# NagsTheProgrammer/WindGNN

Measured on AMD Instinct MI355X. Metric: windows/sec (fwd+bwd) 34-node seq24 GCN-GRU, higher is better.
Workload: dtype f16x3(split-fp32); 1 GPU; S=34 stations, T=24, F=13, H=102, B=4096 windows/GPU; step = forward + MSE + backward + grad all-reduce (N>1) + Adam; fp32 I/O; global_batch=4096, parallelism=dp1, math=f16x3, collective=none (one rank)

## Files before the change

### windgnn_amd/csrc/api.hip

```cpp
#include <atomic>
#include <cmath>
#include <cstdlib>
#include <mutex>

#include "common.h"
#include "../../include/windgnn_optim.h"
#include "../../include/windgnn_sched.h"

namespace {

inline size_t rup(size_t x, size_t a) { return (x + a - 1) / a * a; }

struct Layout {
  size_t BT, I, Ip, G3, Gp, H, Hp;
  size_t Id;
  int np_g3, np_i;
  size_t ws_GI, ws_g, ws_planes_f, ws_Ylast, ws_xtail_f, ws_xtail_b, fwd_floats;
  size_t st_g, st_gates, st_yp, stash_floats;
  size_t ws_dGI, ws_dGH, ws_dg, ws_part_ih, ws_part_hh, ws_gcnpart, ws_planes_b, ws_scales, ws_dY, bwd_floats;
  size_t prep_f, prep_b, prep_floats;
  int prep_kind;
  int sk_ih, sk_hh;
  bool tn_merge;
  bool x3, gen_gcn, gen_gru, g32, g32tn;
  int hq;
  int np_h;
  bool dg16;
  bool gi16;
  bool dgi1;
  bool gen2p;
  bool small, rec32;
  size_t st_hprev;
  bool dghn;
  int hn, msplit, m_hh;
  size_t st_h1;
  size_t st_stats;
  size_t st_GI;
  bool gi_stash;
  size_t ws_gh, ws_h1, ws_yp, ws_hhp_f, ws_kp_f, ws_hc, ws_du, ws_dhz, ws_dhw, ws_hhp_b, ws_kp_b, ws_dc;
  size_t ws_ntk_f, ws_ntk_b;
  size_t ws_aimg_f, ws_aimg_b;
  bool state;
  size_t plane_rows;
  size_t st_h0;
};

int pick_splitk(size_t BT, int tiles, int target_wgs, int min_rows) {
  int by_rows = (int)(BT / (size_t)min_rows);
  int by_grid = target_wgs / (tiles > 0 ? tiles : 1);
  int sk = by_rows < by_grid ? by_rows : by_grid;
  if (sk >= 8) sk -= sk % 8;
  return sk < 1 ? 1 : sk;
}

bool three_pass(const wgnn_dims* d) { return d->math == WGNN_MATH_F16X3 || d->math == WGNN_MATH_F16X3G; }

Layout make_layout(const wgnn_dims* d, bool state = false, int series = SER_NONE ) {
  Layout L;
  L.state = state;
  L.x3 = d->math != WGNN_MATH_F32;
  L.gen_gcn = d->adj_format == WGNN_ADJ_CSR;
  L.gen_gru = L.x3 ? !grux_shape_supported(d->H) : !gru_shape_supported(d->H);
  const bool x3 = L.x3;
  L.BT = (size_t)d->B * d->T;
  L.I = (size_t)d->S * d->F;
  L.Ip = rup(L.I + 1, 32);
  L.Id = rup(L.I, 16);
  L.H = d->H;
  L.Hp = x3 ? (size_t)grux_hp(d->H) : 0;
  L.G3 = 3 * (size_t)d->H;
  L.Gp = rup(L.G3, 32);
  L.np_g3 = pgemm_nt_np((int)L.G3);
  L.np_i = pgemm_nt_np((int)L.I);
  auto al = [](size_t x) { return align_up(x, 64); };
  L.g32 = !x3 && !L.gen_gcn && !L.gen_gru && gemm32_nt_supported(L.BT, (int)L.Ip, (int)L.Gp);
  L.g32tn = L.g32 && gemm32_tn_supported(L.BT);
  L.small = !x3 && !L.gen_gru && !series && gru_small_supported(d->B, d->H);
  L.rec32 = !x3 && !L.gen_gru && !L.small;
  const bool g32_shape = !x3 && !L.gen_gcn && !L.gen_gru && gemm32_nt_supported(1u << 30, (int)L.Ip, (int)L.Gp);
  const size_t planes_f = ser_front(series, x3 ? (size_t)L.np_g3 * L.Ip : (g32_shape ? (size_t)gemm32_nt_rows((int)L.G3) * L.Ip : 0));
  const size_t planes_b = ser_front(series, x3 ? (size_t)L.np_i * L.Gp : (g32_shape ? (size_t)gemm32_nt_rows((int)L.I) * L.Gp : 0));
  L.prep_kind = x3 ? 1 : (g32_shape ? 2 : 0);
  L.prep_f = 0;
  L.prep_b = al(planes_f);
  L.prep_floats = L.prep_kind ? al(planes_f) + al(planes_b) : 0;
  constexpr size_t HDR = WGNN_STATUS_BYTES / sizeof(float);
  size_t o = HDR;
  L.ws_GI = o; o += al(ser_front(series, L.BT * L.Gp));
  L.ws_g = o; o += al(ser_front(series, L.BT * L.Ip));
  L.ws_planes_f = o; o += al(planes_f);
  L.np_h = pgemm_nt_np((int)L.H);
  L.ws_gh = o; o += al(L.gen_gru ? (size_t)d->B * L.Gp : 0);
  L.ws_h1 = o; o += al(L.gen_gcn ? L.BT * L.I : 0);
  L.ws_yp = o; o += al(L.gen_gru && x3 ? (L.BT + 1) * L.Hp : 0);
  L.ws_hhp_f = o; o += al(L.gen_gru && x3 ? (size_t)L.np_g3 * L.Hp : 0);
  L.ws_kp_f = o; o += al(L.gen_gru && x3 ? pgemm_nt_kpart_floats(d->B, (int)L.Gp, (int)L.Hp) : 0);
  L.ws_hc = o; o += al(L.gen_gru && x3 ? (size_t)d->B * L.Hp : 0);
  L.ws_xtail_f = o; o += al(ser_front(series, (L.I & 1) && !L.gen_gcn ? L.I + 1 : 0));
  if ((x3 && !L.gen_gru) || L.rec32 || L.H <= L.Ip) { L.ws_Ylast = L.ws_g; }
  else { L.ws_Ylast = o; o += al(L.BT * L.H); }
  L.ws_aimg_f = o; o += al(x3 ? pgemm_nt256_aimg_bytes((int)L.BT, (int)L.G3, (int)L.Ip, 2) / 4 : 0);
  {
    const int sk = (!x3 && !L.g32 && L.BT < 65536) ? gemm_f32_nt_splitk((int)L.BT, (int)L.G3, (int)L.I) : 1;
    L.ws_ntk_f = o; o += al(ser_front(series, sk > 1 ? (size_t)sk * L.BT * L.G3 : 0));
  }
  L.fwd_floats = o;
  o = 0;
  L.st_g = o; o += al(ser_front(series, L.BT * L.Ip));
  {
    const size_t plain = L.BT * 4 * L.H, grec = (x3 && !L.gen_gru) ? grux_gates_floats(d->B, d->T, d->H, d->io)
                                                                   : (L.rec32 ? gru_gates_floats(d->B, d->T, d->H) : 0);
    L.st_gates = o; o += al(series == SER_FRONT ? 0 : series == SER_REC ? grec : (plain > grec ? plain : grec));
  }
  L.plane_rows = L.BT + (state ? (size_t)d->B : 1);
  L.st_yp = o; o += al(L.plane_rows * L.Hp);
  L.st_h1 = o; o += al(L.gen_gcn ? L.BT * L.I : 0);
  {
    const size_t nb = L.small ? (size_t)gru_small_blocks(d->B) : (size_t)grux_blocks(d->B);
    L.st_stats = o; o += al(series ? 0 : 2 * nb + 4);
  }
  L.gi_stash = (x3 && !L.gen_gru && three_pass(d)) || L.rec32;
  L.st_GI = o; o += al(ser_front(series, L.gi_stash ? L.BT * L.Gp : 0));
  L.hq = (int)rup(L.H + 1, 16);
  const bool hprev_rows = L.g32tn || (state && !x3);
  L.st_hprev = o; o += al(ser_rec(series, hprev_rows ? L.BT * (size_t)L.hq : 0));
  L.st_h0 = o; o += al(state ? (size_t)d->B * L.H : 0);
  L.stash_floats = o;
  L.dghn = (x3 && !L.gen_gru) || (L.rec32 && L.g32tn);
  L.dgi1 = d->math == WGNN_MATH_F16X3G && !L.gen_gru && L.BT >= 4096;
  L.gen2p = d->math == WGNN_MATH_F16X3G && L.gen_gru && L.BT >= 3072;
  L.dg16 = (L.dgi1 || (d->math == WGNN_MATH_F16 && !L.gen_gru)) && !L.gen_gcn;
  L.gi16 = d->math == WGNN_MATH_F16 && !L.gen_gru;
  L.hn = x3 ? grux_hn(d->H) : gru_hn(d->H);
  L.msplit = x3 ? grux_msplit(d->H) : gru_msplit(d->H);
  L.m_hh = L.dghn ? (x3 ? L.msplit + L.hn : L.msplit + (int)L.H) : (int)L.G3;
  if (x3) {
    L.sk_ih = pick_splitk(L.BT, pgemm_tn_tiles((int)L.G3, (int)L.I + 1), 256, 64);
    L.sk_hh = pick_splitk(L.BT, pgemm_tn_tiles(L.m_hh, (int)L.H + 1), 256, 64);
    L.tn_merge = L.dghn;
  } else {
    L.tn_merge = false;
    L.sk_ih = L.g32tn ? pick_splitk(L.BT, gemm32_tn_tiles((int)L.G3, (int)L.I + 1), 256, 64)
                    : pick_splitk(L.BT, gemm_f32_tiles((int)L.G3, (int)L.I + 1), 1024, 128);
    L.sk_hh = L.g32tn ? pick_splitk(L.BT, gemm32_tn_tiles(L.m_hh, (int)L.H + 1), 256, 64)
                    : pick_splitk(L.BT, gemm_f32_tiles((int)L.G3, (int)L.H + 1), 1024, 128);
  }
  size_t part_ih = (size_t)L.sk_ih * L.G3 * (L.g32tn ? (size_t)gemm32_tn_pitch((int)L.I + 1) : L.I + 1);
  size_t part_hh = (size_t)L.sk_hh * (size_t)L.m_hh * (L.g32tn ? (size_t)gemm32_tn_pitch((int)L.H + 1) : L.H + 1);
  if (x3) {
    part_ih = pgemm_tn_partial_floats((int)L.G3, (int)L.I + 1, L.sk_ih);
    part_hh = pgemm_tn_partial_floats(L.m_hh, (int)L.H + 1, L.sk_hh);
  }
  o = HDR;
  L.ws_dGI = o; o += al(L.BT * L.Gp);
  L.ws_dGH = o; o += al(ser_rec(series, L.dghn ? L.BT * (size_t)L.hn : L.BT * L.Gp));
  L.ws_dg = o; o += al(ser_front(series, L.BT * L.Id));
  L.ws_part_ih = o; o += al(ser_front(series, part_ih));
  L.ws_part_hh = o; o += al(ser_rec(series, part_hh));
  {
    size_t a = gcn32_bwd_partial_floats((int)L.BT), b = gcnx2_bwd_partial_floats((int)L.BT);
    if (L.gen_gcn) a = gcn_csr_bwd_partial_floats();
    L.ws_gcnpart = o; o += al(ser_front(series, a > b ? a : b));
  }
  L.ws_du = o; o += al(L.gen_gcn ? L.BT * L.I : 0);
  L.ws_dhz = o; o += al(L.gen_gru ? (size_t)d->B * L.H : 0);
  L.ws_dhw = o; o += al(L.gen_gru ? (size_t)d->B * L.H : 0);
  L.ws_hhp_b = o; o += al(L.gen_gru && x3 ? (size_t)L.np_h * L.Gp : 0);
  L.ws_kp_b = o; o += al(L.gen_gru && x3 ? pgemm_nt_kpart_floats(d->B, (int)L.H, (int)L.Gp) : 0);
  L.ws_dc = o; o += al(L.gen_gru && x3 ? (size_t)d->B * L.Gp : 0);
  L.ws_planes_b = o; o += al(planes_b);
  L.ws_scales = o; o += al(4096);
  L.ws_dY = o; o += al(series ? 0 : L.BT * L.H);
  L.ws_xtail_b = o; o += al(ser_front(series, (L.I & 1) && !L.gen_gcn ? L.I + 1 : 0));
  L.ws_aimg_b = o; o += al(x3 ? pgemm_nt256_aimg_bytes((int)L.BT, (int)L.I, (int)L.Gp, 2) / 4 : 0);
  {
    const int sk = (!x3 && !L.g32 && L.BT < 65536) ? gemm_f32_nt_splitk((int)L.BT, (int)L.I, (int)L.G3) : 1;
    L.ws_ntk_b = o; o += al(ser_front(series, sk > 1 ? (size_t)sk * L.BT * L.I : 0));
  }
  L.bwd_floats = o;
  return L;
}

template <class P>
void slots(const P& s, float* out[8]) {
  const float* v[8] = {s.conv1_weight, s.conv1_bias, s.conv2_weight, s.conv2_bias, s.w_ih, s.w_hh, s.b_ih, s.b_hh};
  for (int t = 0; t < 8; ++t) out[t] = const_cast<float*>(v[t]);
}

template <class P>
bool complete(const P& s, bool conv = true) {
  float* v[8];
  slots(s, v);
  for (int t = conv ? 0 : 4; t < 8; ++t)
    if (!v[t]) return false;
  return true;
}

bool overlap(const void* a, size_t na, const void* b, size_t nb) {
  return a && b && (const char*)a < (const char*)b + nb && (const char*)b < (const char*)a + na;
}

template <class Args>
void set_adam(Args& a, const wgnn_adam* adam) {
  const double bc1 = 1.0 - pow((double)adam->beta1, (double)adam->step);
  const double bc2 = 1.0 - pow((double)adam->beta2, (double)adam->step);
  a.lr_over_bc1 = (float)(adam->lr / bc1);
  a.inv_sqrt_bc2 = (float)(1.0 / sqrt(bc2));
  a.b1 = adam->beta1; a.b2 = adam->beta2; a.eps = adam->eps;
}

template <class Args>
void set_planes(Args& a, const Layout& L, void* prepared) {
  a.pf_hi = (_Float16*)((float*)prepared + L.prep_f); a.pf_lo = a.pf_hi + (size_t)L.np_g3 * L.Ip;
  a.pb_hi = (_Float16*)((float*)prepared + L.prep_b); a.pb_lo = a.pb_hi + (size_t)L.np_i * L.Gp;
  a.np_g3 = L.np_g3; a.np_i = L.np_i;
}

void fill_reduce(const Layout& L, const wgnn_dims* d, const wgnn_grads* g, float* ws, int which, FinishArgs& a) {
  a.scales = ws + L.ws_scales;
  a.status = (unsigned*)ws;
  slots(*g, a.g);
  const int F = d->F;
  const int64_t n[8] = {(int64_t)F * F, F, (int64_t)F * F, F, (int64_t)L.G3 * (int64_t)L.I, (int64_t)L.G3 * (int64_t)L.H,
                        (int64_t)L.G3, (int64_t)L.G3};
  for (int t = 0; t < 8; ++t) a.n[t] = (int)n[t];
  a.I = (int)L.I;
  if (which & 4) {
    FinSeg& ih = a.ih;
    ih.partial = ws + L.ws_part_ih;
    ih.splitk = L.sk_ih;
    ih.kind = L.x3 ? 2 : 1;
    ih.Mout = ih.Mgemm = (int)L.G3; ih.Nout = (int)L.I + 1; ih.ncols = (int)L.I;
    ih.scaled = L.x3;
    FinSeg& hh = a.hh;
    hh = ih;
    hh.partial = ws + L.ws_part_hh;
    hh.splitk = L.sk_hh;
    hh.Nout = (int)L.H + 1; hh.ncols = (int)L.H;
    hh.Mgemm = L.m_hh;
    ih.pitch = L.g32tn ? gemm32_tn_pitch(ih.Nout) : ih.Nout;
    hh.pitch = L.g32tn ? gemm32_tn_pitch(hh.Nout) : hh.Nout;
    if (L.dghn) { hh.msplit = L.msplit; hh.rows1 = 2 * d->H; }
    if (L.x3) {
      pgemm_tn_geom((int)L.G3, ih.Nout, &ih.T, &ih.nNb, &ih.ntiles);
      pgemm_tn_geom(L.m_hh, hh.Nout, &hh.T, &hh.nNb, &hh.ntiles);
    }
  }
  if (which & 2) {
    a.conv_partial = ws + L.ws_gcnpart;
    a.conv_rows = L.gen_gcn ? gcn_csr_bwd_rows()
                            : (L.x3 ? gcnx_bwd_grid((int)L.BT, d->S, three_pass(d)) : gcn32_bwd_grid((int)L.BT, d->S));
  }
}

void fill_adam(const Layout& L, const wgnn_params* p, const wgnn_adam* adam, FinishArgs& a) {
  slots(*p, a.p);
  slots(adam->exp_avg, a.m);
  slots(adam->exp_avg_sq, a.v);
  a.adam = 1;
  set_adam(a, adam);
  if (p->prepared && L.prep_kind) {
    a.prep_kind = L.prep_kind;
    if (L.prep_kind == 1) {
      set_planes(a, L, p->prepared);
    } else {
      a.wp = (float*)p->prepared + L.prep_f;
      a.wt = (float*)p->prepared + L.prep_b;
    }
    a.Ip = (int)L.Ip; a.Gp = (int)L.Gp;
  }
}

void fill_norm(const Layout& L, const wgnn_dims* d, const wgnn_grads* g, float* ws, int which, FinishArgs& a) {
  fill_reduce(L, d, g, ws, which, a);
  a.elem_mask = ((which & 4) ? 0u : 0xF0u) | ((which & 2) ? 0u : 0x0Fu);
}

size_t clip_floats(const Layout& L, const wgnn_dims* d) {
  const wgnn_grads none = {};
  float* const nowhere = reinterpret_cast<float*>((uintptr_t)WGNN_STATUS_BYTES);
  int64_t most = 0;
  for (int which = 0; which <= 6; which += 2) {
    FinishArgs a = {};
    fill_norm(L, d, &none, nowhere, which, a);
    int64_t grid;
    if (finish_grid(a, &grid) != WGNN_OK) return 0;
    most = grid > most ? grid : most;
  }
  return rup((size_t)CLIP_HDR + (size_t)most, 64);
}

std::atomic<int> g_opt[WGNN_OPT_COUNT];
std::once_flag g_opt_once;

int env_int(const char* name, int dflt, int lo, int hi) {
  const char* e = getenv(name);
  if (!e || !e[0]) return dflt;
  char* end = nullptr;
  const long v = strtol(e, &end, 10);
  return (end == e || v < lo || v > hi) ? dflt : (int)v;
}

void init_options() {
  std::call_once(g_opt_once, [] {
    for (int k = 0; k < WGNN_OPT_COUNT; ++k) g_opt[k].store(0, std::memory_order_relaxed);
    g_opt[WGNN_OPT_FUSED_FWD].store(env_int("WGNN_FUSED_FWD", 1, 0, 2), std::memory_order_relaxed);
    g_opt[WGNN_OPT_BIG_GEMM].store(1, std::memory_order_relaxed);
    g_opt[WGNN_OPT_TN_MERGED].store(1, std::memory_order_relaxed);
  });
}

int opt(int key) {
  init_options();
  return g_opt[key].load(std::memory_order_relaxed);
}

bool known_option(int key) { return key == WGNN_OPT_FUSED_FWD || key == WGNN_OPT_BIG_GEMM || key == WGNN_OPT_TN_MERGED; }

int check_dims(const wgnn_dims* d) {
  if (!d) return WGNN_ERR_NULL;
  if (d->B < 1 || d->T < 1 || d->S < 1 || d->H < 1) return WGNN_ERR_SHAPE;
  if (d->F != 13) return WGNN_ERR_SHAPE;
  if ((int64_t)d->B * d->T > (1 << 30)) return WGNN_ERR_SHAPE;
  if (d->math != WGNN_MATH_F32 && d->math != WGNN_MATH_F16X3 && d->math != WGNN_MATH_F16 && d->math != WGNN_MATH_F16X3G)
    return WGNN_ERR_DTYPE;
  if (d->io != WGNN_IO_F32 && d->io != WGNN_IO_F16 && d->io != WGNN_IO_BF16) return WGNN_ERR_DTYPE;
  if (d->io != WGNN_IO_F32 &&
      (d->math == WGNN_MATH_F32 || d->adj_format != WGNN_ADJ_DENSE || d->S > 64 || !grux_shape_supported(d->H)))
    return WGNN_ERR_UNSUPPORTED;
  if (d->adj_format == WGNN_ADJ_CSR) {
    if (d->nnz < 1 || (int64_t)d->nnz > (int64_t)d->S * d->S) return WGNN_ERR_SHAPE;
  } else if (d->adj_format == WGNN_ADJ_DENSE) {
    if (d->S > 64) return WGNN_ERR_UNSUPPORTED;
  } else {
    return WGNN_ERR_UNSUPPORTED;
  }
  if ((int64_t)3 * d->H * d->S * d->F >= (1ll << 31) || (int64_t)3 * d->H * d->H >= (1ll << 31)) return WGNN_ERR_SHAPE;
  if ((int64_t)d->B * d->T * d->S * d->F >= (1ll << 31) || (int64_t)d->B * d->T * 4 * d->H >= (1ll << 31))
    return WGNN_ERR_SHAPE;
  return WGNN_OK;
}

struct FwdCall {
  const float* A = nullptr;
  const void* X = nullptr;
  const float* g_in = nullptr;
  const wgnn_params* p = nullptr;
  const void* labels = nullptr;
  const float* h0 = nullptr;
  void* Y = nullptr;
  float* hn = nullptr;
  float* last = nullptr;
  float wind_min = 0.f, wind_max = 1.f;
  void* stash = nullptr;
  bool state = false, sst = false;
  void* workspace;
  size_t workspace_bytes;
  void* stream;
  FwdCall(void* ws, size_t ws_bytes, void* st) : workspace(ws), workspace_bytes(ws_bytes), stream(st) {}
};

struct Fwd {
  const wgnn_dims* d;
  const FwdCall& c;
  const Layout& L;
  hipStream_t st = (hipStream_t)c.stream;
  float* ws = (float*)c.workspace;
  unsigned* status = (unsigned*)c.workspace;
  float* sf = (float*)c.stash;
  float* GI = (sf && L.gi_stash) ? sf + L.st_GI : ws + L.ws_GI;
  float* g = sf ? sf + L.st_g : ws + L.ws_g;
  float* gates = sf ? sf + L.st_gates : nullptr;
  bool full = three_pass(d);
  bool kept = c.p->prepared != nullptr && L.prep_kind != 0;
  float* img_f = kept ? (float*)c.p->prepared + L.prep_f : ws + L.ws_planes_f;
  bool reg = (L.x3 && !L.gen_gru) || L.rec32;
  void* Y = (!reg && (c.last || (c.state && !c.Y))) ? ws + L.ws_Ylast : c.Y;
};

int fwd_front(const Fwd& f) {
  const wgnn_dims* d = f.d;
  const FwdCall& c = f.c;
  const Layout& L = f.L;
  const wgnn_params* p = c.p;
  const int fmode = opt(WGNN_OPT_FUSED_FWD);
  int rc;
  if (c.g_in) {
    rc = launch_pack_g(c.g_in, L.BT, (int)L.I, f.g, (int)L.Ip, f.st);
  } else if (L.x3 && !L.gen_gcn && !L.gen_gru && (fmode == 2 || (fmode == 1 && !f.sf)) && gcngi_supported(d->S, d->H, f.full)) {
    const int planes = f.sf ? ((f.full && !L.dgi1) ? 2 : 1) : 0;
    return launch_gcngi_fwd((int)L.BT, d->S, c.A, c.X, d->io, p->conv1_weight, p->conv1_bias, p->conv2_weight, p->conv2_bias,
                            f.sf ? (void*)f.g : nullptr, (int)L.Ip, planes, f.img_f, L.np_g3, f.GI, (int)L.Gp, (int)L.G3, f.full,
                            f.status, f.ws + L.ws_xtail_f, f.st);
  } else if (L.gen_gcn) {
    rc = launch_gcn2_csr_fwd((int)L.BT, d->S, d->nnz, c.A, (const float*)c.X, p->conv1_weight, p->conv1_bias, p->conv2_weight,
                             p->conv2_bias, f.sf ? f.sf + L.st_h1 : f.ws + L.ws_h1, L.x3 ? nullptr : f.g, L.x3 ? f.g : nullptr,
                             L.Ip, f.full, L.x3 ? f.status : nullptr, f.st);
  } else if (L.x3) {
    rc = launch_gcnx2_fwd((int)L.BT, d->S, c.A, c.X, d->io, p->conv1_weight, p->conv1_bias, p->conv2_weight, p->conv2_bias, f.g,
                          (int)L.Ip, f.full, f.status, f.ws + L.ws_xtail_f, f.st);
  } else {
    rc = launch_gcn32_fwd((int)L.BT, d->S, c.A, (const float*)c.X, p->conv1_weight, p->conv1_bias, p->conv2_weight,
                          p->conv2_bias, f.g, (int)L.Ip, f.ws + L.ws_xtail_f, f.st);
  }
  if (rc != WGNN_OK) return rc;
  if (L.x3) {
    const _Float16* ghi = (const _Float16*)f.g;
    const size_t aimg_f = pgemm_nt256_aimg_bytes((int)L.BT, (int)L.G3, (int)L.Ip, 2);
    return launch_pgemm_nt(ghi, ghi + L.BT * L.Ip, (int)L.Ip, (int)L.BT, (int)L.Ip, f.img_f, L.np_g3, f.GI, (int)L.Gp,
                           (int)L.G3, nullptr, f.full, nullptr, f.st, L.gi16, aimg_f ? f.ws + L.ws_aimg_f : nullptr);
  }
  if (L.g32) {
    if (!f.kept) {
      rc = launch_pad_weight(p->w_ih, (int)L.G3, (int)L.I, 0, p->b_ih, f.img_f, gemm32_nt_rows((int)L.G3), (int)L.Ip, f.st);
      if (rc != WGNN_OK) return rc;
    }
    return launch_gemm32_nt(f.g, (int)L.Ip, (int)L.BT, (int)L.Ip, f.img_f, f.GI, (int)L.Gp, (int)L.G3, f.st);
  }
  GemmArgs ga = {};
  ga.A = f.g; ga.lda = (int)L.Ip; ga.a_kcontig = 1;
  ga.B = p->w_ih; ga.ldb = (int)L.I; ga.b_kcontig = 1;
  ga.C = f.GI; ga.ldc = (int)L.Gp; ga.M = (int)L.BT; ga.N = (int)L.G3; ga.K = (int)L.I;
  ga.bias = p->b_ih; ga.splitk = 1;
  return launch_gemm_f32_nt(ga, gemm_f32_nt_splitk(ga.M, ga.N, ga.K) > 1 && L.BT < 65536 ? f.ws + L.ws_ntk_f : nullptr, f.st);
}

int fwd_recurrence(const Fwd& f) {
  const wgnn_dims* d = f.d;
  const FwdCall& c = f.c;
  const Layout& L = f.L;
  const wgnn_params* p = c.p;
  const float y_mul = c.wind_max - c.wind_min, y_add = c.wind_min;
  const bool hn_only = c.state && !f.Y;
  float* Y = (float*)f.Y;
  const void* labels = f.sf ? c.labels : nullptr;
  float* stats = f.sf ? f.sf + L.st_stats : nullptr;
  float* hprev = (f.sf && (L.g32tn || c.sst)) ? f.sf + L.st_hprev : nullptr;
  int rc;
  if (L.x3 && !L.gen_gru) {
    if (c.last)
      return launch_grux_fwd(d->B, d->T, d->H, f.GI, (int)L.Gp, p->w_hh, p->b_hh, c.last, nullptr, nullptr, f.full, f.status,
                             nullptr, nullptr, 0, 1, y_mul, y_add, f.st);
    if (c.state) {
      const int lo = hn_only && d->io == WGNN_IO_F32;
      return launch_grux_fwd(d->B, d->T, d->H, f.GI, (int)L.Gp, p->w_hh, p->b_hh, lo ? (void*)c.hn : f.Y, nullptr, nullptr,
                             f.full, f.status, nullptr, nullptr, d->io, lo, 1.f, 0.f, f.st, c.h0, lo ? nullptr : c.hn);
    }
    rc = launch_grux_fwd(d->B, d->T, d->H, f.GI, (int)L.Gp, p->w_hh, p->b_hh, f.Y, f.gates,
                         f.sf && !hh_from_y(d, L.tn_merge, c.sst) ? f.sf + L.st_yp : nullptr, f.full, f.status, labels, stats,
                         d->io, 0, 1.f, 0.f, f.st, c.h0, c.hn, c.sst ? L.plane_rows : 0);
  } else if (L.rec32) {
    if (c.last)
      return launch_gru_fwd(d->B, d->T, d->H, f.GI, (int)L.Gp, p->w_hh, p->b_hh, c.last, nullptr, nullptr, nullptr, nullptr, 0,
                            1, y_mul, y_add, f.st);
    if (c.state)
      return launch_gru_fwd(d->B, d->T, d->H, f.GI, (int)L.Gp, p->w_hh, p->b_hh, hn_only ? c.hn : Y, nullptr, nullptr, nullptr,
                            nullptr, 0, hn_only ? 1 : 0, 1.f, 0.f, f.st, c.h0, hn_only ? nullptr : c.hn);
    rc = launch_gru_fwd(d->B, d->T, d->H, f.GI, (int)L.Gp, p->w_hh, p->b_hh, Y, f.gates, (const float*)labels, stats, hprev,
                        L.hq, 0, 1.f, 0.f, f.st, c.h0, c.hn);
  } else if (L.small) {
    rc = launch_gru_small_fwd(d->B, d->T, d->H, f.GI, (int)L.Gp, p->w_hh, p->b_hh, Y, f.gates, hprev, L.hq,
                              (const float*)labels, stats, f.st, c.h0, c.hn);
  } else if (L.x3) {
    rc = launch_split_weight2(p->w_hh, (int)L.G3, (int)L.H, 0, p->b_hh, (int)L.H, f.ws + L.ws_hhp_f, L.np_g3, (int)L.Hp,
                              f.status, f.st);
    if (rc == WGNN_OK)
      rc = launch_gru_gen_fwd_x3(d->B, d->T, d->H, f.GI, (int)L.Gp, f.ws + L.ws_hhp_f, L.np_g3, p->b_hh, Y, f.gates,
                                 f.sf ? f.sf + L.st_yp : f.ws + L.ws_yp, f.ws + L.ws_gh, f.ws + L.ws_kp_f, f.ws + L.ws_hc,
                                 f.full, f.st, c.h0, c.sst ? L.plane_rows : 0);
  } else {
    rc = launch_gru_gen_fwd(d->B, d->T, d->H, f.GI, (int)L.Gp, p->w_hh, p->b_hh, Y, f.gates, f.ws + L.ws_gh, f.st, c.h0);
  }
  if (rc != WGNN_OK) return rc;
  const size_t h4 = (size_t)d->H * 4;
  if (L.gen_gru && c.hn &&
      hipMemcpy2DAsync(c.hn, h4, Y + (size_t)(d->T - 1) * d->H, d->T * h4, h4, d->B, hipMemcpyDeviceToDevice, f.st) != hipSuccess)
    return WGNN_ERR_HIP;
  if (c.sst) {
    const float* h0c = f.sf + L.st_h0;
    if (L.x3) {
      _Float16* yh = (_Float16*)(f.sf + L.st_yp);
      return launch_h0_planes(d->B, d->H, (int)L.Hp, h0c, yh + L.BT * L.Hp, yh + (L.plane_rows + L.BT) * L.Hp, f.st);
    }
    float* hp = f.sf + L.st_hprev;
    const size_t hq4 = (size_t)L.hq * 4;
    if (L.gen_gru && L.BT > 1 &&
        hipMemcpy2DAsync(hp + L.hq, hq4, Y, h4, h4, L.BT - 1, hipMemcpyDeviceToDevice, f.st) != hipSuccess)
      return WGNN_ERR_HIP;
    return hipMemcpy2DAsync(hp, (size_t)d->T * hq4, h0c, h4, h4, d->B, hipMemcpyDeviceToDevice, f.st) == hipSuccess ? WGNN_OK
                                                                                                              : WGNN_ERR_HIP;
  }
  if (c.last)
    return wgnn_predict_last(Y, d->B, d->T, d->H, c.wind_min, c.wind_max, c.last, c.stream);
  return WGNN_OK;
}

int fwd(const wgnn_dims* d, const FwdCall& c) {
  int rc = check_dims(d);
  if (rc != WGNN_OK) return rc;
  if ((!c.g_in && (!c.A || !c.X)) || !c.p || (!c.Y && !c.last && !(c.state && c.hn)) || (c.sst && !c.stash) || !c.workspace)
    return WGNN_ERR_NULL;
  if (!complete(*c.p, !c.g_in)) return WGNN_ERR_NULL;
  if (c.g_in && (d->math != WGNN_MATH_F32 || d->io != WGNN_IO_F32 || d->adj_format != WGNN_ADJ_DENSE)) return WGNN_ERR_UNSUPPORTED;
  const size_t hb = (size_t)d->B * d->H * sizeof(float), yb = (size_t)d->B * d->T * d->H * (d->io == WGNN_IO_F32 ? 4 : 2);
  if (overlap(c.h0, hb, c.hn, hb) || overlap(c.h0, hb, c.Y, yb) || overlap(c.Y, yb, c.hn, hb)) return WGNN_ERR_UNSUPPORTED;
  const Layout L = make_layout(d, c.sst);
  if (c.workspace_bytes < sizeof(float) * L.fwd_floats) return WGNN_ERR_WORKSPACE;
  const wgnn_params* p = c.p;
  hipStream_t st = (hipStream_t)c.stream;
  if (c.state && d->T == 1 && d->adj_format == WGNN_ADJ_DENSE && d->io == WGNN_IO_F32 && gru_step_supported(d->B, d->S, d->H))
    return launch_gru_step(d->B, d->S, d->H, c.A, (const float*)c.X, p->conv1_weight, p->conv1_bias, p->conv2_weight,
                           p->conv2_bias, p->w_ih, p->b_ih, p->w_hh, p->b_hh, c.h0, (float*)c.Y, c.hn, st);
  const Fwd f{d, c, L};
  if (c.sst &&
      (c.h0 ? hipMemcpyAsync(f.sf + L.st_h0, c.h0, hb, hipMemcpyDeviceToDevice, st)
            : hipMemsetAsync(f.sf + L.st_h0, 0, hb, st)) != hipSuccess)
    return WGNN_ERR_HIP;
  if (L.x3 && !f.kept) {
    rc = launch_split_weight2(p->w_ih, (int)L.G3, (int)L.I, 0, p->b_ih, (int)L.I, f.img_f, L.np_g3, (int)L.Ip, f.status, st);
    if (rc != WGNN_OK) return rc;
  }
  rc = fwd_front(f);
  if (rc != WGNN_OK) return rc;
  return fwd_recurrence(f);
}

struct BwdCall {
  const float* A = nullptr;
  const void* X = nullptr;
  const wgnn_params* p = nullptr;
  const void* Y = nullptr;
  const float* dY = nullptr;
  const void* labels = nullptr;
  float grad_scale = 1.f;
  float* loss = nullptr;
  const void* stash = nullptr;
  const wgnn_grads* g = nullptr;
  int part = 0;
  float* dg_out = nullptr;
  bool sst = false;
  const float* dhn = nullptr;
  float* dh0 = nullptr;
  void* workspace;
  size_t workspace_bytes;
  void* stream;
  BwdCall(void* ws, size_t ws_bytes, void* st) : workspace(ws), workspace_bytes(ws_bytes), stream(st) {}
};

struct Bwd {
  const wgnn_dims* d;
  const BwdCall& c;
  const Layout& L;
  hipStream_t st = (hipStream_t)c.stream;
  float* ws = (float*)c.workspace;
  unsigned* status = (unsigned*)c.workspace;
  const float* sf = (const float*)c.stash;
  const float* Y = (const float*)c.Y;
  const float* gact = sf + L.st_g;
  float* dGI = ws + L.ws_dGI;
  float* dGH = ws + L.ws_dGH;
  float* dg = ws + L.ws_dg;
  float* scales = ws + L.ws_scales;
  bool full = three_pass(d);
  bool defer = c.part & WGNN_BWD_DEFER;
  bool stats_ready = (c.part & 8) && c.labels;
  bool fused_loss = c.labels && ((L.x3 && !L.gen_gru) || ((L.rec32 || L.small) && stats_ready));
};

int bwd_rec(const Bwd& b) {
  const wgnn_dims* d = b.d;
  const BwdCall& c = b.c;
  const Layout& L = b.L;
  const wgnn_params* p = c.p;
  const float* labels = (const float*)c.labels;
  const float* gates = b.sf + L.st_gates;
  const float* stats = b.fused_loss && b.stats_ready ? b.sf + L.st_stats : nullptr;
  const BwdState sbs = {c.sst ? b.sf + L.st_h0 : nullptr, c.dhn, c.dh0};
  const BwdState* sb = c.sst ? &sbs : nullptr;
  const float* dY = c.dY;
  int rc;
  if (labels && !b.fused_loss) {
    rc = launch_mse(b.Y, labels, (int64_t)L.BT * L.H, c.grad_scale, b.ws + L.ws_dY, c.loss, b.scales + 64, b.st);
    if (rc != WGNN_OK) return rc;
    dY = b.ws + L.ws_dY;
  }
  if (L.x3) {
    if (b.fused_loss && b.stats_ready)
      rc = WGNN_OK;
    else if (b.fused_loss)
      rc = launch_mse_stats(b.Y, labels, (int64_t)L.BT * L.H, c.grad_scale, c.loss, b.scales, b.scales + 64, b.st);
    else
      rc = launch_amax_scale(dY, (int64_t)L.BT * L.H, b.scales, b.scales + 64, b.st,
                             c.dhn, c.dhn ? (int64_t)d->B * d->H : 0);
    if (rc != WGNN_OK) return rc;
    if (L.gen_gru) {
      rc = launch_split_weight2(p->w_hh, (int)L.G3, (int)L.H, 1, nullptr, 0, b.ws + L.ws_hhp_b, L.np_h, (int)L.Gp, b.status,
                                b.st);
      if (rc != WGNN_OK) return rc;
      return launch_gru_gen_bwd_x3(d->B, d->T, d->H, b.ws + L.ws_hhp_b, L.np_h, b.Y, dY, gates, b.scales, b.dGI, b.dGH,
                                   (int)L.Gp, b.ws + L.ws_dhz, b.ws + L.ws_dhw, b.ws + L.ws_kp_b, b.ws + L.ws_dc, b.full, b.st, sb);
    }
    return launch_grux_bwd(d->B, d->T, d->H, p->w_hh, c.Y, b.fused_loss ? nullptr : dY, b.fused_loss ? c.labels : nullptr,
                           d->io, gates, L.gi_stash ? b.sf + L.st_GI : nullptr, (int)L.Gp, b.scales, b.dGI, b.dGH, (int)L.Gp,
                           b.full, stats, (int64_t)L.BT * L.H, c.grad_scale, c.loss, b.scales, b.status, L.dgi1 ? 0 : 1, b.st,
                           sb);
  }
  if (L.gen_gru)
    return launch_gru_gen_bwd(d->B, d->T, d->H, p->w_hh, b.Y, dY, gates, b.dGI, b.dGH, (int)L.Gp, b.ws + L.ws_dhz,
                              b.ws + L.ws_dhw, b.st, sb);
  if (L.small)
    return launch_gru_small_bwd(d->B, d->T, d->H, p->w_hh, b.Y, b.fused_loss ? nullptr : dY, b.fused_loss ? labels : nullptr,
                                gates, b.dGI, b.dGH, (int)L.Gp, stats, (int64_t)L.BT * L.H, c.grad_scale, c.loss, b.status,
                                b.st, sb);
  return launch_gru_bwd(d->B, d->T, d->H, p->w_hh, b.Y, b.fused_loss ? nullptr : dY, b.fused_loss ? labels : nullptr, gates,
                        b.sf + L.st_GI, (int)L.Gp, b.dGI, (int)L.Gp, L.dghn ? b.dGH : nullptr, L.dghn ? nullptr : b.dGH, stats,
                        (int64_t)L.BT * L.H, c.grad_scale, c.loss, b.status, b.st, sb);
}

int bwd_weights(const Bwd& b, int prods, int r0, int rows) {
  const wgnn_dims* d = b.d;
  const Layout& L = b.L;
  float* part_ih = b.ws + L.ws_part_ih;
  float* part_hh = b.ws + L.ws_part_hh;
  const bool sst = b.c.sst;
  int rc = WGNN_OK;
  if (L.x3) {
    const _Float16* dGIh = (const _Float16*)b.dGI + r0;
    const _Float16* dGHh = (const _Float16*)b.dGH + r0;
    const _Float16* gh = (const _Float16*)b.gact;
    const _Float16 *yph = (const _Float16*)(b.sf + L.st_yp), *ypl = yph + L.plane_rows * L.Hp;
    const size_t PG = L.BT * L.Gp;
    TnProd hh = {};
    hh.lda = (int)L.Gp; hh.Bhi = yph; hh.Blo = ypl; hh.ldb = (int)L.Hp; hh.shift_T = d->T; hh.splitk = L.sk_hh;
    hh.partial = part_hh; hh.Nout = (int)L.H + 1; hh.x3 = b.full; hh.per_window = sst;
    if (L.dghn) {
      hh.Ahi = dGIh; hh.Alo = L.dgi1 ? nullptr : dGIh + PG; hh.Mout = L.m_hh;
      hh.A2hi = dGHh; hh.A2lo = L.dgi1 ? nullptr : dGHh + L.BT * (size_t)L.hn; hh.lda2 = L.hn; hh.msplit = L.msplit;
      hh.b_stream = true;
    } else {
      hh.Ahi = dGHh; hh.Alo = L.gen2p ? nullptr : dGHh + PG; hh.Mout = rows;
    }
    const bool one_pass_ih = L.dgi1 || L.gen2p;
    TnProd ih = {};
    ih.Ahi = dGIh; ih.Alo = one_pass_ih ? dGIh : dGIh + PG; ih.lda = (int)L.Gp;
    ih.Bhi = gh; ih.Blo = gh + L.BT * L.Ip; ih.ldb = (int)L.Ip; ih.splitk = L.sk_ih;
    ih.partial = part_ih; ih.Mout = rows; ih.Nout = (int)L.I + 1; ih.x3 = b.full && !one_pass_ih; ih.b_stream = true;
    auto one = [&](const TnProd& p) {
      return launch_pgemm_tn(p.Ahi, p.Alo, p.lda, p.Bhi, p.Blo, p.ldb, p.shift_T, (int)L.BT, p.splitk, p.partial, p.Mout, p.Nout,
                             p.x3, p.A2hi, p.A2lo, p.lda2, p.msplit, b.st, p.b_stream, p.per_window);
    };
    if (prods == (WGNN_ROWS_IH | WGNN_ROWS_HH) && L.tn_merge && opt(WGNN_OPT_TN_MERGED) && pgemm_tn2_covers(ih, hh)) {
      rc = launch_pgemm_tn2(ih, tn_b_from_y(hh, hh_from_y(d, L.tn_merge, sst) ? b.Y : nullptr, (int)L.H), (int)L.BT, b.st);
    } else {
      if (prods & WGNN_ROWS_HH) {
        rc = one(hh);
        if (rc != WGNN_OK) return rc;
      }
      if (prods & WGNN_ROWS_IH) rc = one(ih);
    }
  } else {
    const float* hp = b.sf + L.st_hprev;
    if (prods & WGNN_ROWS_HH) {
      if (L.g32tn && L.dghn)
        rc = launch_gemm32_tn(b.dGI, (int)L.Gp, hp, L.hq, (int)L.BT, L.sk_hh, part_hh, L.m_hh, (int)L.H + 1, b.dGH, L.hn,
                              L.msplit, b.st);
      else if (L.g32tn)
        rc = launch_gemm32_tn(b.dGH, (int)L.Gp, hp, L.hq, (int)L.BT, L.sk_hh, part_hh, rows, (int)L.H + 1, nullptr, 0, 0, b.st);
      else {
        GemmArgs a = {};
        a.A = b.dGH + r0; a.lda = (int)L.Gp; a.a_kcontig = 0;
        a.B = b.Y; a.ldb = (int)L.H; a.b_kcontig = 0; a.ones_col = 1; a.shift_T = d->T;
        if (sst) { a.B = hp; a.ldb = L.hq; a.shift_T = 0; }
        a.M = rows; a.N = (int)L.H + 1; a.K = (int)L.BT;
        a.splitk = L.sk_hh; a.partial = part_hh;
        rc = launch_gemm_f32(a, b.st);
      }
      if (rc != WGNN_OK) return rc;
    }
    if (prods & WGNN_ROWS_IH) {
      if (L.g32tn) {
        rc = launch_gemm32_tn(b.dGI, (int)L.Gp, b.gact, (int)L.Ip, (int)L.BT, L.sk_ih, part_ih, rows, (int)L.I + 1, nullptr, 0,
                              0, b.st);
      } else {
        GemmArgs a = {};
        a.A = b.dGI + r0; a.lda = (int)L.Gp; a.a_kcontig = 0;
        a.B = b.gact; a.ldb = (int)L.Ip; a.b_kcontig = 0; a.ones_col = 1;
        a.M = rows; a.N = (int)L.I + 1; a.K = (int)L.BT;
        a.splitk = L.sk_ih; a.partial = part_ih;
        rc = launch_gemm_f32(a, b.st);
      }
    }
  }
  if (rc != WGNN_OK || b.defer) return rc;
  FinishArgs a = {};
  fill_reduce(L, d, b.c.g, b.ws, 4, a);
  if (prods != (WGNN_ROWS_IH | WGNN_ROWS_HH)) {
    const bool ih = prods == WGNN_ROWS_IH;
    FinSeg& s = ih ? a.ih : a.hh;
    (ih ? a.hh : a.ih) = FinSeg{};
    if (rows != (int)L.G3) {
      s.Mout = s.Mgemm = rows;
      if (L.x3) pgemm_tn_geom(rows, s.Nout, &s.T, &s.nNb, &s.ntiles);
    }
    a.g[ih ? 4 : 5] += (size_t)r0 * s.ncols;
    a.g[ih ? 6 : 7] += r0;
  }
  return launch_finish(a, b.st);
}

int bwd_dg(const Bwd& b) {
  const wgnn_dims* d = b.d;
  const BwdCall& c = b.c;
  const Layout& L = b.L;
  const wgnn_params* p = c.p;
  const bool kept = p->prepared != nullptr && L.prep_kind != 0;
  float* img_b = kept ? (float*)p->prepared + L.prep_b : b.ws + L.ws_planes_b;
  int rc;
  if (L.x3) {
    if (!kept) {
      rc = launch_split_weight2(p->w_ih, (int)L.G3, (int)L.I, 1, nullptr, 0, img_b, L.np_i, (int)L.Gp, b.status, b.st);
      if (rc != WGNN_OK) return rc;
    }
    const _Float16* dGIh = (const _Float16*)b.dGI;
    const size_t aimg_b = pgemm_nt256_aimg_bytes((int)L.BT, (int)L.I, (int)L.Gp, 2);
    rc = launch_pgemm_nt(dGIh, (L.dgi1 || L.gen2p) ? nullptr : dGIh + L.BT * L.Gp, (int)L.Gp, (int)L.BT, (int)L.Gp, img_b,
                         L.np_i, b.dg, (int)L.Id, (int)L.I, nullptr, b.full, nullptr, b.st, L.dg16,
                         aimg_b ? b.ws + L.ws_aimg_b : nullptr);
  } else if (L.g32) {
    if (!kept) {
      rc = launch_pad_weight(p->w_ih, (int)L.G3, (int)L.I, 1, nullptr, img_b, gemm32_nt_rows((int)L.I), (int)L.Gp, b.st);
      if (rc != WGNN_OK) return rc;
    }
    rc = launch_gemm32_nt(b.dGI, (int)L.Gp, (int)L.BT, (int)L.Gp, img_b, b.dg, (int)L.Id, (int)L.I, b.st);
  } else {
    GemmArgs a = {};
    a.A = b.dGI; a.lda = (int)L.Gp; a.a_kcontig = 1;
    a.B = p->w_ih; a.ldb = (int)L.I; a.b_kcontig = 0;
    a.C = b.dg; a.ldc = (int)L.Id; a.M = (int)L.BT; a.N = (int)L.I; a.K = (int)L.G3; a.splitk = 1;
    rc = launch_gemm_f32_nt(a, gemm_f32_nt_splitk(a.M, a.N, a.K) > 1 && L.BT < 65536 ? b.ws + L.ws_ntk_b : nullptr, b.st);
  }
  if (rc != WGNN_OK) return rc;
  if (c.dg_out) return launch_unpack_dg(b.dg, L.BT, (int)L.I, (int)L.Id, c.dg_out, b.st);
  if (L.gen_gcn)
    rc = launch_gcn2_csr_bwd((int)L.BT, d->S, d->nnz, c.A, (const float*)c.X, p->conv2_weight, b.sf + L.st_h1,
                             L.x3 ? nullptr : b.gact, L.x3 ? b.gact : nullptr, L.Ip, b.dg, L.Id, L.x3 ? b.scales : nullptr,
                             b.ws + L.ws_du, b.ws + L.ws_gcnpart, nullptr, nullptr, nullptr, nullptr, b.st);
  else if (L.x3)
    rc = launch_gcnx2_bwd((int)L.BT, d->S, c.A, c.X, d->io, p->conv1_weight, p->conv1_bias, p->conv2_weight, b.gact, (int)L.Ip,
                          b.dg, (int)L.Id, L.dg16, b.scales, 0, b.ws + L.ws_gcnpart, b.full, b.ws + L.ws_xtail_b,
                          b.st);
  else
    rc = launch_gcn32_bwd((int)L.BT, d->S, c.A, (const float*)c.X, p->conv1_weight, p->conv1_bias, p->conv2_weight, b.gact,
                          (int)L.Ip, b.dg, (int)L.Id, nullptr, nullptr, nullptr, nullptr, b.ws + L.ws_gcnpart,
                          b.ws + L.ws_xtail_b, b.st);
  if (rc != WGNN_OK || b.defer) return rc;
  FinishArgs a = {};
  fill_reduce(L, d, c.g, b.ws, 2, a);
  return launch_finish(a, b.st);
}

int bwd(const wgnn_dims* d, const BwdCall& c) {
  const int which = c.part;
  if (which < 1 || which > 31 || (which & 7) == 0) return WGNN_ERR_SHAPE;
  int rc = check_dims(d);
  if (rc != WGNN_OK) return rc;
  if ((!c.dg_out && (!c.A || !c.X)) || !c.p || !c.Y || (!c.dY && !c.labels) || !c.stash || !c.g || !c.workspace)
    return WGNN_ERR_NULL;
  if (c.labels && (which & 1) && !c.loss) return WGNN_ERR_NULL;
  if (!complete(*c.g, !c.dg_out)) return WGNN_ERR_NULL;
  if (c.dg_out && (d->math != WGNN_MATH_F32 || d->io != WGNN_IO_F32 || d->adj_format != WGNN_ADJ_DENSE || which != 7))
    return WGNN_ERR_UNSUPPORTED;
  const Layout L = make_layout(d, c.sst);
  if (c.workspace_bytes < sizeof(float) * L.bwd_floats) return WGNN_ERR_WORKSPACE;
  const Bwd b{d, c, L};
  if (d->io != WGNN_IO_F32 && c.labels && (which & 1) && !(b.fused_loss && b.stats_ready)) return WGNN_ERR_UNSUPPORTED;
  if (which & 1) {
    rc = bwd_rec(b);
    if (rc != WGNN_OK) return rc;
  }
  if (which & 4) {
    rc = bwd_weights(b, WGNN_ROWS_IH | WGNN_ROWS_HH, 0, (int)L.G3);
    if (rc != WGNN_OK) return rc;
  }
  return (which & 2) ? bwd_dg(b) : WGNN_OK;
}

int rows_align(const wgnn_dims* d, const Layout& L) {
  if (!L.gen_gru || d->math == WGNN_MATH_F16) return 0;
  return L.x3 ? TN_BM : 128;
}

int check_rows(const wgnn_dims* d, const Layout& L, int which, int row0, int rows) {
  if ((which & ~(WGNN_ROWS_IH | WGNN_ROWS_HH | WGNN_ROWS_STATE)) != 0 ||
      ((which & 3) != WGNN_ROWS_IH && (which & 3) != WGNN_ROWS_HH))
    return WGNN_ERR_SHAPE;
  if (which & WGNN_ROWS_STATE) return WGNN_ERR_UNSUPPORTED;
  const int al = rows_align(d, L);
  if (al == 0) return WGNN_ERR_UNSUPPORTED;
  const int64_t end = (int64_t)row0 + rows;
  if (row0 < 0 || rows < 1 || end > (int64_t)L.G3 || row0 % al != 0 || (end % al != 0 && end != (int64_t)L.G3))
    return WGNN_ERR_SHAPE;
  return WGNN_OK;
}

}

int opt_big_gemm() { return opt(WGNN_OPT_BIG_GEMM); }

bool hh_from_y(const wgnn_dims* d, bool tn_merge, bool sst) {
  static const int from_env = env_int("WGNN_TN_YFP32", 1, 0, 1);
  return tn_merge && three_pass(d) && d->io == WGNN_IO_F32 && !sst && from_env && opt(WGNN_OPT_TN_MERGED);
}

int series_plan(const wgnn_dims* df, const wgnn_dims* dr, SeriesPlan* sp) {
  int rc = check_dims(df);
  if (rc == WGNN_OK) rc = check_dims(dr);
  if (rc != WGNN_OK) return rc;
  const Layout Lf = make_layout(df, false, SER_FRONT), Lr = make_layout(dr, false, SER_REC);
  if ((int64_t)Lf.BT * (int64_t)Lf.Gp >= (1ll << 31)) return WGNN_ERR_SHAPE;
  sp->ws_front = Lf.fwd_floats > Lf.bwd_floats ? Lf.fwd_floats : Lf.bwd_floats;
  sp->ws_rec = Lr.fwd_floats > Lr.bwd_floats ? Lr.fwd_floats : Lr.bwd_floats;
  sp->ws_front_fwd = Lf.fwd_floats;
  sp->st_front = Lf.stash_floats;
  sp->st_rec = Lr.stash_floats;
  sp->st_g = Lf.BT * Lf.Ip; sp->st_GI = Lf.BT * Lf.Gp;
  sp->st_gates = gru_gates_floats(dr->B, dr->T, dr->H);
  sp->st_hprev = Lr.g32tn ? Lr.BT * (size_t)Lr.hq : 0;
  return WGNN_OK;
}

namespace {

int series_forward(const wgnn_dims* df, const wgnn_dims* dr, int stride, const float* A, const float* Xs, const wgnn_params* p,
                   float* Y, float* last, float wind_min, float wind_max, void* stash, void* workspace, const SeriesPlan& sp,
                   void* stream, const float* Ls, int64_t ls_rows, float* loss_buf, const int* starts, bool masked = false,
                   const LossFn* lossfn = nullptr) {
  const int last_start = df->T - dr->T;
  const Layout Lf = make_layout(df, false, SER_FRONT), Lr = make_layout(dr, false, SER_REC);
  FwdCall cf(workspace, sizeof(float) * sp.ws_front, stream);
  cf.A = A; cf.X = Xs; cf.p = p; cf.stash = stash;
  const Fwd f{df, cf, Lf};
  int rc = fwd_front(f);
  if (rc != WGNN_OK) return rc;
  hipStream_t st = (hipStream_t)stream;
  const int ld = (int)Lf.Gp;
  if (last)
    return launch_gru_fwd(dr->B, dr->T, dr->H, f.GI, ld, p->w_hh, p->b_hh, last, nullptr, nullptr, nullptr, nullptr, 0, 1,
                          wind_max - wind_min, wind_min, st, nullptr, nullptr, stride, 0, starts, last_start);
  float* sr = stash ? (float*)stash + sp.st_front : nullptr;
  return launch_gru_fwd(dr->B, dr->T, dr->H, f.GI, ld, p->w_hh, p->b_hh, Y, sr ? sr + Lr.st_gates : nullptr, Ls, loss_buf,
                        sr && Lr.g32tn ? sr + Lr.st_hprev : nullptr, Lr.hq, 0, 1.f, 0.f, st, nullptr, nullptr, stride, ls_rows,
                        starts, last_start, masked, lossfn);
}

int series_backward(const wgnn_dims* df, const wgnn_dims* dr, int stride, const float* A, const float* Xs, const wgnn_params* p,
                    const float* Y, const float* dY, const void* stash, const wgnn_grads* g, void* workspace, const SeriesPlan& sp,
                    void* stream, const float* Ls, int64_t ls_rows, float grad_scale, const float* loss_buf, float* loss,
                    const int* starts, bool masked = false, const LossFn* lossfn = nullptr) {
  const Layout Lf = make_layout(df, false, SER_FRONT), Lr = make_layout(dr, false, SER_REC);
  const float* sff = (const float*)stash;
  BwdCall cr((float*)workspace + sp.ws_front, sizeof(float) * sp.ws_rec, stream);
  cr.p = p; cr.Y = Y; cr.dY = dY; cr.stash = sff + sp.st_front; cr.g = g; cr.part = 7;
  const Bwd br{dr, cr, Lr};
  BwdCall cf(workspace, sizeof(float) * sp.ws_front, stream);
  cf.A = A; cf.X = Xs; cf.p = p; cf.Y = Y; cf.dY = dY; cf.stash = stash; cf.g = g; cf.part = 7;
  const Bwd bf{df, cf, Lf};
  int rc = launch_gru_bwd(dr->B, dr->T, dr->H, p->w_hh, Y, dY, Ls, br.sf + Lr.st_gates, sff + Lf.st_GI, (int)Lf.Gp, br.dGI,
                          (int)Lr.Gp, Lr.dghn ? br.dGH : nullptr, Lr.dghn ? nullptr : br.dGH, loss_buf, (int64_t)Lr.BT * Lr.H,
                          grad_scale, loss, Ls ? br.status : nullptr, br.st, nullptr, stride, ls_rows, starts,
                          df->T - dr->T, masked, lossfn);
  if (rc != WGNN_OK) return rc;
  rc = bwd_weights(br, WGNN_ROWS_HH, 0, (int)Lr.G3);
  if (rc != WGNN_OK) return rc;
  rc = starts ? launch_series_fold_at(br.dGI, starts, dr->B, dr->T, df->T, (int)Lf.G3, (int)Lf.Gp, bf.dGI, bf.st)
              : launch_series_fold(br.dGI, dr->B, dr->T, stride, df->T, (int)Lf.G3, (int)Lf.Gp, bf.dGI, bf.st);
  if (rc != WGNN_OK) return rc;
  rc = bwd_weights(bf, WGNN_ROWS_IH, 0, (int)Lf.G3);
  if (rc != WGNN_OK) return rc;
  return bwd_dg(bf);
}

}

int series_fwd(const wgnn_dims* df, const wgnn_dims* dr, int stride, const float* A, const float* Xs, const wgnn_params* p,
               float* Y, float* last, float wind_min, float wind_max, void* stash, void* workspace, const SeriesPlan& sp,
               void* stream, const int* starts) {
  return series_forward(df, dr, stride, A, Xs, p, Y, last, wind_min, wind_max, stash, workspace, sp, stream, nullptr, 0, nullptr,
                        starts);
}

int series_bwd(const wgnn_dims* df, const wgnn_dims* dr, int stride, const float* A, const float* Xs, const wgnn_params* p,
               const float* Y, const float* dY, const void* stash, const wgnn_grads* g, void* workspace, const SeriesPlan& sp,
               void* stream, const int* starts) {
  return series_backward(df, dr, stride, A, Xs, p, Y, dY, stash, g, workspace, sp, stream, nullptr, 0, 1.f, nullptr, nullptr,
                         starts);
}

size_t series_loss_floats(int n) { return 2 * (size_t)gru_blocks(n) + 4; }
size_t series_masked_loss_floats(int n) { return series_loss_floats(n) + (size_t)gru_blocks(n); }

int series_fwd_loss(const wgnn_dims* df, const wgnn_dims* dr, int stride, const float* A, const float* Xs, const wgnn_params* p,
                    const float* Ls, int64_t ls_rows, float* Y, void* stash, float* loss_buf, void* workspace,
                    const SeriesPlan& sp, void* stream, const int* starts, bool masked, const LossFn* lossfn) {
  return series_forward(df, dr, stride, A, Xs, p, Y, nullptr, 0.f, 1.f, stash, workspace, sp, stream, Ls, ls_rows, loss_buf,
                        starts, masked, lossfn);
}

int series_bwd_mse(const wgnn_dims* df, const wgnn_dims* dr, int stride, const float* A, const float* Xs, const wgnn_params* p,
                   const float* Y, const float* Ls, int64_t ls_rows, float grad_scale, const void* stash, const float* loss_buf,
                   float* loss, const wgnn_grads* g, void* workspace, const SeriesPlan& sp, void* stream, const int* starts,
                   bool masked, const LossFn* lossfn) {
  return series_backward(df, dr, stride, A, Xs, p, Y, nullptr, stash, g, workspace, sp, stream, Ls, ls_rows, grad_scale, loss_buf,
                         loss, starts, masked, lossfn);
}

int series_val_fwd(const wgnn_dims* df, const wgnn_dims* dr, int stride, const float* A, const float* Xs, const wgnn_params* p,
                   const float* Ls, int64_t ls_rows, float* last, float wind_min, float wind_max, float* loss_buf,
                   void* workspace, const SeriesPlan& sp, void* stream, const int* starts, const LossFn* lossfn) {
  const Layout Lf = make_layout(df, false, SER_FRONT);
  FwdCall cf(workspace, sizeof(float) * sp.ws_front_fwd, stream);
  cf.A = A; cf.X = Xs; cf.p = p;
  const Fwd f{df, cf, Lf};
  int rc = fwd_front(f);
  if (rc != WGNN_OK) return rc;
  return launch_gru_fwd(dr->B, dr->T, dr->H, f.GI, (int)Lf.Gp, p->w_hh, p->b_hh, last, nullptr, Ls, loss_buf, nullptr, 0, 1,
                        wind_max - wind_min, wind_min, (hipStream_t)stream, nullptr, nullptr, stride, ls_rows, starts,
                        df->T - dr->T, false, lossfn);
}

extern "C" {

int wgnn_version(void) { return WGNN_VERSION; }

int wgnn_get_option(int key) { return known_option(key) ? opt(key) : WGNN_ERR_SHAPE; }

int wgnn_set_option(int key, int value) {
  if (!known_option(key)) return WGNN_ERR_SHAPE;
  if (key == WGNN_OPT_FUSED_FWD && (value < 0 || value > 2)) return WGNN_ERR_SHAPE;
  if ((key == WGNN_OPT_BIG_GEMM || key == WGNN_OPT_TN_MERGED) && (value < 0 || value > 1)) return WGNN_ERR_SHAPE;
  init_options();
  return g_opt[key].exchange(value, std::memory_order_relaxed);
}

const char* wgnn_strerror(int status) {
  switch (status) {
    case WGNN_OK: return "ok";
    case WGNN_ERR_NULL: return "required pointer is NULL";
    case WGNN_ERR_SHAPE: return "invalid shape (need B,T,S,H >= 1 and F == 13)";
    case WGNN_ERR_DTYPE: return "unsupported dtype / math mode";
    case WGNN_ERR_WORKSPACE: return "workspace or stash too small";
    case WGNN_ERR_UNSUPPORTED:
      return "configuration not supported by this build (a dense adjacency needs S <= 64: pass larger graphs as CSR)";
    case WGNN_ERR_HIP: return "HIP runtime error (kernel launch failed)";
    case WGNN_ERR_RANGE:
      return "a value left fp16's range in an fp16-plane math mode (status block bits: 1 activation, 2 weight, 4 "
             "non-finite gradient): normalise the inputs or use WGNN_MATH_F32; or (bit 8) the backward was told the "
             "forward's loss statistics are in the stash but the last forward on it was not wgnn_fwd_loss";
    default: return "unknown status";
  }
}

size_t wgnn_workspace_bytes(const wgnn_dims* d) {
  if (check_dims(d) != WGNN_OK) return 0;
  Layout L = make_layout(d);
  return sizeof(float) * (L.fwd_floats > L.bwd_floats ? L.fwd_floats : L.bwd_floats);
}

size_t wgnn_stash_bytes(const wgnn_dims* d) {
  if (check_dims(d) != WGNN_OK) return 0;
  return sizeof(float) * make_layout(d).stash_floats;
}

size_t wgnn_state_stash_bytes(const wgnn_dims* d) {
  if (check_dims(d) != WGNN_OK) return 0;
  return sizeof(float) * make_layout(d, true).stash_floats;
}

size_t wgnn_prepared_bytes(const wgnn_dims* d) {
  if (check_dims(d) != WGNN_OK) return 0;
  return sizeof(float) * make_layout(d).prep_floats;
}

int wgnn_fwd(const wgnn_dims* d, const float* A, const void* X, const wgnn_params* p, void* Y, void* stash,
             void* workspace, size_t workspace_bytes, void* stream) {
  FwdCall c(workspace, workspace_bytes, stream);
  c.A = A; c.X = X; c.p = p; c.Y = Y; c.stash = stash;
  return fwd(d, c);
}

int wgnn_fwd_loss(const wgnn_dims* d, const float* A, const void* X, const wgnn_params* p, const void* labels,
                  void* Y, void* stash, void* workspace, size_t workspace_bytes, void* stream) {
  if (!labels || !stash) return WGNN_ERR_NULL;
  FwdCall c(workspace, workspace_bytes, stream);
  c.A = A; c.X = X; c.p = p; c.labels = labels; c.Y = Y; c.stash = stash;
  return fwd(d, c);
}

int wgnn_fwd_last(const wgnn_dims* d, const float* A, const void* X, const wgnn_params* p, float wind_min,
                  float wind_max, float* out, void* workspace, size_t workspace_bytes, void* stream) {
  if (!out) return WGNN_ERR_NULL;
  if (d && d->io != WGNN_IO_F32) return WGNN_ERR_UNSUPPORTED;
  FwdCall c(workspace, workspace_bytes, stream);
  c.A = A; c.X = X; c.p = p; c.last = out; c.wind_min = wind_min; c.wind_max = wind_max;
  return fwd(d, c);
}

int wgnn_fwd_state(const wgnn_dims* d, const float* A, const void* X, const wgnn_params* p, const float* h0, void* Y,
                   float* h_n, void* workspace, size_t workspace_bytes, void* stream) {
  FwdCall c(workspace, workspace_bytes, stream);
  c.A = A; c.X = X; c.p = p; c.h0 = h0; c.Y = Y; c.hn = h_n; c.state = true;
  return fwd(d, c);
}

int wgnn_fwd_state_stash(const wgnn_dims* d, const float* A, const void* X, const wgnn_params* p, const float* h0, void* Y,
                         float* h_n, void* stash, void* workspace, size_t workspace_bytes, void* stream) {
  FwdCall c(workspace, workspace_bytes, stream);
  c.A = A; c.X = X; c.p = p; c.h0 = h0; c.Y = Y; c.hn = h_n; c.stash = stash; c.sst = true;
  return fwd(d, c);
}

int wgnn_gru_fwd(const wgnn_dims* d, const float* g, const wgnn_params* p, void* Y, void* stash, void* workspace,
                 size_t workspace_bytes, void* stream) {
  if (!g) return WGNN_ERR_NULL;
  FwdCall c(workspace, workspace_bytes, stream);
  c.g_in = g; c.p = p; c.Y = Y; c.stash = stash;
  return fwd(d, c);
}

int wgnn_prepare_weights(const wgnn_dims* d, const wgnn_params* p, void* workspace, size_t workspace_bytes,
                         void* stream) {
  int rc = check_dims(d);
  if (rc != WGNN_OK) return rc;
  if (!p || !p->w_ih || !p->b_ih || !p->prepared || !workspace) return WGNN_ERR_NULL;
  if (workspace_bytes < WGNN_STATUS_BYTES) return WGNN_ERR_WORKSPACE;
  const Layout L = make_layout(d);
  if (L.prep_kind == 0) return WGNN_ERR_UNSUPPORTED;
  hipStream_t st = (hipStream_t)stream;
  float* img_f = (float*)p->prepared + L.prep_f;
  float* img_b = (float*)p->prepared + L.prep_b;
  if (L.prep_kind == 1) {
    rc = launch_split_weight2(p->w_ih, (int)L.G3, (int)L.I, 0, p->b_ih, (int)L.I, img_f, L.np_g3, (int)L.Ip,
                              (unsigned*)workspace, st);
    if (rc != WGNN_OK) return rc;
    return launch_split_weight2(p->w_ih, (int)L.G3, (int)L.I, 1, nullptr, 0, img_b, L.np_i, (int)L.Gp, (unsigned*)workspace, st);
  }
  rc = launch_pad_weight(p->w_ih, (int)L.G3, (int)L.I, 0, p->b_ih, img_f, gemm32_nt_rows((int)L.G3), (int)L.Ip, st);
  if (rc != WGNN_OK) return rc;
  return launch_pad_weight(p->w_ih, (int)L.G3, (int)L.I, 1, nullptr, img_b, gemm32_nt_rows((int)L.I), (int)L.Gp, st);
}

int wgnn_bwd(const wgnn_dims* d, const float* A, const void* X, const wgnn_params* p, const void* Y,
             const float* dY, const void* stash, const wgnn_grads* g, void* workspace, size_t workspace_bytes,
             void* stream) {
  return wgnn_bwd_part(d, A, X, p, Y, dY, stash, g, workspace, workspace_bytes, stream, 7);
}

int wgnn_bwd_part(const wgnn_dims* d, const float* A, const void* X, const wgnn_params* p, const void* Y,
                  const float* dY, const void* stash, const wgnn_grads* g, void* workspace, size_t workspace_bytes,
                  void* stream, int which) {
  if (!dY) return WGNN_ERR_NULL;
  BwdCall c(workspace, workspace_bytes, stream);
  c.A = A; c.X = X; c.p = p; c.Y = Y; c.dY = dY; c.stash = stash; c.g = g; c.part = which;
  return bwd(d, c);
}

int wgnn_bwd_mse_part(const wgnn_dims* d, const float* A, const void* X, const wgnn_params* p, const void* Y,
                      const void* labels, float grad_scale, float* loss, const void* stash, const wgnn_grads* g,
                      void* workspace, size_t workspace_bytes, void* stream, int which) {
  if (!labels) return WGNN_ERR_NULL;
  BwdCall c(workspace, workspace_bytes, stream);
  c.A = A; c.X = X; c.p = p; c.Y = Y; c.labels = labels; c.grad_scale = grad_scale; c.loss = loss; c.stash = stash; c.g = g;
  c.part = which;
  return bwd(d, c);
}

int wgnn_bwd_state_part(const wgnn_dims* d, const float* A, const void* X, const wgnn_params* p, const void* Y,
                        const float* dY, const float* dh_n, const void* stash, const wgnn_grads* g, float* dh0,
                        void* workspace, size_t workspace_bytes, void* stream, int part) {
  int rc = check_dims(d);
  if (rc != WGNN_OK) return rc;
  if (!dY) return WGNN_ERR_NULL;
  const size_t hb = (size_t)d->B * d->H * sizeof(float), yb = (size_t)d->B * d->T * d->H * sizeof(float);
  if (overlap(dh0, hb, dh_n, hb) || overlap(dh0, hb, dY, yb) || overlap(dh0, hb, stash, wgnn_state_stash_bytes(d)))
    return WGNN_ERR_UNSUPPORTED;
  BwdCall c(workspace, workspace_bytes, stream);
  c.A = A; c.X = X; c.p = p; c.Y = Y; c.dY = dY; c.stash = stash; c.g = g; c.part = part;
  c.sst = true; c.dhn = dh_n; c.dh0 = dh0;
  return bwd(d, c);
}

int wgnn_gru_bwd(const wgnn_dims* d, const float* g, const wgnn_params* p, const void* Y, const float* dY, const void* stash,
                 const wgnn_grads* grads, float* dg, void* workspace, size_t workspace_bytes, void* stream) {
  if (!g || !dY || !dg) return WGNN_ERR_NULL;
  BwdCall c(workspace, workspace_bytes, stream);
  c.p = p; c.Y = Y; c.dY = dY; c.stash = stash; c.g = grads; c.part = 7; c.dg_out = dg;
  return bwd(d, c);
}

int wgnn_bwd_rows_align(const wgnn_dims* d) {
  if (check_dims(d) != WGNN_OK) return 0;
  return rows_align(d, make_layout(d));
}

int wgnn_bwd_rows(const wgnn_dims* d, const void* Yv, const void* stash, const wgnn_grads* g, int which, int row0, int rows,
                  void* workspace, size_t workspace_bytes, void* stream) {
  int rc = check_dims(d);
  if (rc != WGNN_OK) return rc;
  if (!Yv || !stash || !g || !workspace) return WGNN_ERR_NULL;
  const bool ih = (which & 3) == WGNN_ROWS_IH;
  if (ih ? (!g->w_ih || !g->b_ih) : (!g->w_hh || !g->b_hh)) return WGNN_ERR_NULL;
  const Layout L = make_layout(d);
  rc = check_rows(d, L, which, row0, rows);
  if (rc != WGNN_OK) return rc;
  if (workspace_bytes < sizeof(float) * L.bwd_floats) return WGNN_ERR_WORKSPACE;
  BwdCall c(workspace, workspace_bytes, stream);
  c.Y = Yv; c.stash = stash; c.g = g;
  return bwd_weights(Bwd{d, c, L}, which & 3, row0, rows);
}

int wgnn_finish(const wgnn_dims* d, const wgnn_params* p, const wgnn_grads* g, int which, const wgnn_adam* adam,
                void* workspace, size_t workspace_bytes, void* stream) {
  int rc = check_dims(d);
  if (rc != WGNN_OK) return rc;
  const int only = which & (WGNN_FINISH_ADAM_GRU | WGNN_FINISH_ADAM_CONV);
  if ((which & ~(6 | WGNN_FINISH_ADAM_GRU | WGNN_FINISH_ADAM_CONV)) != 0 || (which == 0 && !adam)) return WGNN_ERR_SHAPE;
  if (only && (!adam || (which & 6) != 0 || only == (WGNN_FINISH_ADAM_GRU | WGNN_FINISH_ADAM_CONV))) return WGNN_ERR_SHAPE;
  if (!g || !workspace || (adam && !p)) return WGNN_ERR_NULL;
  if (!complete(*g)) return WGNN_ERR_NULL;
  const Layout L = make_layout(d);
  if (workspace_bytes < sizeof(float) * L.bwd_floats) return WGNN_ERR_WORKSPACE;
  FinishArgs a = {};
  fill_reduce(L, d, g, (float*)workspace, which, a);
  if (adam) {
    if (!complete(*p)) return WGNN_ERR_NULL;
    if (adam->step < 1) return WGNN_ERR_SHAPE;
    if (!complete(adam->exp_avg) || !complete(adam->exp_avg_sq)) return WGNN_ERR_NULL;
    fill_adam(L, p, adam, a);
    a.elem_mask = ((which & 4) ? 0u : 0xF0u) | ((which & 2) ? 0u : 0x0Fu);
    if (only == WGNN_FINISH_ADAM_GRU) a.elem_mask = 0xF0u;
    if (only == WGNN_FINISH_ADAM_CONV) a.elem_mask = 0x0Fu;
  }
  return launch_finish(a, (hipStream_t)stream);
}

int wgnn_optim_version(void) { return WGNN_OPTIM_VERSION; }

int wgnn_tn_split(const wgnn_dims* d, int state, wgnn_tn_split_info* out) {
  int rc = check_dims(d);
  if (rc != WGNN_OK) return rc;
  if (!out) return WGNN_ERR_NULL;
  const Layout L = make_layout(d, state != 0);
  out->sk_ih = L.sk_ih;
  out->sk_hh = L.sk_hh;
  out->kchunk_ih = cdiv_i(cdiv_i((int)L.BT, L.sk_ih), 32) * 32;
  out->kchunk_hh = cdiv_i(cdiv_i((int)L.BT, L.sk_hh), 32) * 32;
  out->merged = L.tn_merge ? 1 : 0;
  out->workgroups = 0;
  if (L.x3) {
    const int ni = L.sk_ih * pgemm_tn_tiles((int)L.G3, (int)L.I + 1), nh = L.sk_hh * pgemm_tn_tiles(L.m_hh, (int)L.H + 1);
    out->workgroups = L.tn_merge ? (ni > nh ? ni : nh) : ni + nh;
  }
  return WGNN_OK;
}

size_t wgnn_clip_bytes(const wgnn_dims* d) {
  if (check_dims(d) != WGNN_OK) return 0;
  return sizeof(float) * clip_floats(make_layout(d), d);
}

int wgnn_finish_norm(const wgnn_dims* d, const wgnn_grads* g, int which, float max_norm, void* clip, void* workspace,
                     size_t workspace_bytes, void* stream) {
  int rc = check_dims(d);
  if (rc != WGNN_OK) return rc;
  if ((which & ~6) != 0 || !(max_norm > 0.f)) return WGNN_ERR_SHAPE;
  if (!g || !clip || !workspace) return WGNN_ERR_NULL;
  if (!complete(*g)) return WGNN_ERR_NULL;
  const Layout L = make_layout(d);
  if (workspace_bytes < sizeof(float) * L.bwd_floats) return WGNN_ERR_WORKSPACE;
  FinishArgs a = {};
  fill_norm(L, d, g, (float*)workspace, which, a);
  a.clip = (float*)clip;
  a.max_norm = max_norm;
  int64_t grid;
  if (finish_grid(a, &grid) != WGNN_OK || (size_t)CLIP_HDR + (size_t)grid > clip_floats(L, d)) return WGNN_ERR_SHAPE;
  return launch_finish_norm(a, (hipStream_t)stream);
}

int wgnn_finish_clipped(const wgnn_dims* d, const wgnn_params* p, const wgnn_grads* g, const wgnn_adam* adam, const void* clip,
                        void* workspace, size_t workspace_bytes, void* stream) {
  int rc = check_dims(d);
  if (rc != WGNN_OK) return rc;
  if (!p || !g || !adam || !clip || !workspace) return WGNN_ERR_NULL;
  if (!complete(*g) || !complete(*p) || !complete(adam->exp_avg) || !complete(adam->exp_avg_sq)) return WGNN_ERR_NULL;
  if (adam->step < 1) return WGNN_ERR_SHAPE;
  const Layout L = make_layout(d);
  if (workspace_bytes < sizeof(float) * L.bwd_floats) return WGNN_ERR_WORKSPACE;
  FinishArgs a = {};
  fill_norm(L, d, g, (float*)workspace, 0, a);
  fill_adam(L, p, adam, a);
  a.clip = const_cast<float*>((const float*)clip);
  return launch_finish_clipped(a, (hipStream_t)stream);
}

int wgnn_finish_rows(const wgnn_dims* d, const wgnn_params* p, const wgnn_grads* g, int which, int row0, int rows,
                     const wgnn_adam* adam, void* workspace, size_t workspace_bytes, void* stream) {
  int rc = check_dims(d);
  if (rc != WGNN_OK) return rc;
  if (!p || !g || !adam || !workspace) return WGNN_ERR_NULL;
  const Layout L = make_layout(d);
  rc = check_rows(d, L, which, row0, rows);
  if (rc != WGNN_OK) return rc;
  if (adam->step < 1) return WGNN_ERR_SHAPE;
  if (workspace_bytes < WGNN_STATUS_BYTES) return WGNN_ERR_WORKSPACE;
  const bool ih = (which & 3) == WGNN_ROWS_IH;
  const wgnn_grads& m = adam->exp_avg;
  const wgnn_grads& v = adam->exp_avg_sq;
  RowsAdamArgs r = {};
  r.ncols = ih ? (int)L.I : (int)L.H;
  const size_t off = (size_t)row0 * r.ncols;
  r.p_w = const_cast<float*>(ih ? p->w_ih : p->w_hh);
  r.m_w = ih ? m.w_ih : m.w_hh;
  r.v_w = ih ? v.w_ih : v.w_hh;
  r.g_w = ih ? g->w_ih : g->w_hh;
  r.p_b = const_cast<float*>(ih ? p->b_ih : p->b_hh);
  r.m_b = ih ? m.b_ih : m.b_hh;
  r.v_b = ih ? v.b_ih : v.b_hh;
  r.g_b = ih ? g->b_ih : g->b_hh;
  if (!r.p_w || !r.m_w || !r.v_w || !r.g_w || !r.p_b || !r.m_b || !r.v_b || !r.g_b) return WGNN_ERR_NULL;
  r.p_w += off; r.m_w += off; r.v_w += off; r.g_w += off;
  r.p_b += row0; r.m_b += row0; r.v_b += row0; r.g_b += row0;
  r.row0 = row0;
  r.rows = rows;
  set_adam(r, adam);
  r.status = (unsigned*)workspace;
  if (ih && p->prepared && L.prep_kind == 1) set_planes(r, L, p->prepared);
  return launch_adam_rows(r, (hipStream_t)stream);
}

static int gcn_layer_route(int32_t ntiles, int32_t S, int32_t F, int32_t F_out, bool* wide) {
  if (ntiles < 1 || S < 1 || F < 1 || F_out < 1) return WGNN_ERR_SHAPE;
  *wide = F > 64 || F_out > 64;
  if (*wide && !gcn_wide_countable(ntiles, S, F, F_out)) return WGNN_ERR_SHAPE;
  if (!(*wide ? gcn_wide_supported(S, F, F_out) : gcn_any_supported(S, F, F_out))) return WGNN_ERR_UNSUPPORTED;
  return WGNN_OK;
}

size_t wgnn_gcn_layer_workspace_bytes(int32_t ntiles, int32_t S, int32_t F, int32_t F_out) {
  bool wide = false;
  if (gcn_layer_route(ntiles, S, F, F_out, &wide) != WGNN_OK) return 0;
  if (wide) return sizeof(float) * gcn_wide_bwd_ws_floats(ntiles, S, F, F_out);
  if (F == 13 && F_out == 13) return sizeof(float) * gcn1_bwd_partial_floats(ntiles);
  return sizeof(float) * gcn_any_bwd_partial_floats(ntiles, F, F_out);
}

int wgnn_gcn_layer_fwd(int32_t ntiles, int32_t S, int32_t F, int32_t F_out, const float* A, const float* X, const float* W,
                       const float* b, float* out, void* stream) {
  bool wide = false;
  const int rc = gcn_layer_route(ntiles, S, F, F_out, &wide);
  if (rc != WGNN_OK) return rc;
  if (!A || !X || !W || !b || !out) return WGNN_ERR_NULL;
  if (wide) return launch_gcn_wide_fwd(ntiles, S, F, F_out, A, X, W, b, out, (hipStream_t)stream);
  if (F == 13 && F_out == 13) return launch_gcn1_fwd(ntiles, S, A, X, W, b, out, (hipStream_t)stream);
  return launch_gcn_any_fwd(ntiles, S, F, F_out, A, X, W, b, out, (hipStream_t)stream);
}

int wgnn_gcn_layer_bwd(int32_t ntiles, int32_t S, int32_t F, int32_t F_out, const float* A, const float* X, const float* W,
                       const float* out, const float* dout, float* dW, float* db, float* dX, void* workspace,
                       size_t workspace_bytes, void* stream) {
  bool wide = false;
  const int rc = gcn_layer_route(ntiles, S, F, F_out, &wide);
  if (rc != WGNN_OK) return rc;
  if (!A || !X || !W || !out || !dout || !dW || !db || !workspace) return WGNN_ERR_NULL;
  if (workspace_bytes < wgnn_gcn_layer_workspace_bytes(ntiles, S, F, F_out)) return WGNN_ERR_WORKSPACE;
  if (wide)
    return launch_gcn_wide_bwd(ntiles, S, F, F_out, A, X, W, out, dout, dW, db, dX, (float*)workspace, (hipStream_t)stream);
  if (F == 13 && F_out == 13)
    return launch_gcn1_bwd(ntiles, S, A, X, W, out, dout, dW, db, dX, (float*)workspace, (hipStream_t)stream);
  return launch_gcn_any_bwd(ntiles, S, F, F_out, A, X, W, out, dout, dW, db, dX, (float*)workspace, (hipStream_t)stream);
}

size_t wgnn_gcn_layer_csr_workspace_bytes(int32_t ntiles, int32_t S, int32_t F) {
  if (ntiles < 1 || S < 1 || F != 13 || (int64_t)ntiles * S * F >= (1ll << 31)) return 0;
  return sizeof(float) * gcn1_csr_bwd_ws_floats(ntiles, S);
}

int wgnn_gcn_layer_csr_fwd(int32_t ntiles, int32_t S, int32_t F, int32_t nnz, const void* csr, const float* X,
                           const float* W, const float* b, float* out, void* stream) {
  if (ntiles < 1 || S < 1 || F != 13 || nnz < 1 || (int64_t)ntiles * S * F >= (1ll << 31)) return WGNN_ERR_SHAPE;
  if (!csr || !X || !W || !b || !out) return WGNN_ERR_NULL;
  return launch_gcn1_csr_fwd(ntiles, S, nnz, csr, X, W, b, out, (hipStream_t)stream);
}

int wgnn_gcn_layer_csr_bwd(int32_t ntiles, int32_t S, int32_t F, int32_t nnz, const void* csr, const float* X,
                           const float* W, const float* out, const float* dout, float* dW, float* db, float* dX,
                           void* workspace, size_t workspace_bytes, void* stream) {
  if (ntiles < 1 || S < 1 || F != 13 || nnz < 1 || (int64_t)ntiles * S * F >= (1ll << 31)) return WGNN_ERR_SHAPE;
  if (!csr || !X || !W || !out || !dout || !dW || !db || !workspace) return WGNN_ERR_NULL;
  if (workspace_bytes < wgnn_gcn_layer_csr_workspace_bytes(ntiles, S, F)) return WGNN_ERR_WORKSPACE;
  return launch_gcn1_csr_bwd(ntiles, S, nnz, csr, X, W, out, dout, dW, db, dX, (float*)workspace, (hipStream_t)stream);
}

int wgnn_mse_loss_grad(const float* Y, const float* L, int64_t n, float grad_scale, float* dY, float* loss,
                       void* workspace, size_t workspace_bytes, void* stream) {
  if (!Y || !L || !loss || !workspace) return WGNN_ERR_NULL;
  if (n < 1) return WGNN_ERR_SHAPE;
  if (workspace_bytes < 4096) return WGNN_ERR_WORKSPACE;
  return launch_mse(Y, L, n, grad_scale, dY, loss, (float*)workspace, (hipStream_t)stream);
}

int wgnn_adam_step(float* param, const float* grad, float* exp_avg, float* exp_avg_sq, int64_t n, int32_t step,
                   float lr, float beta1, float beta2, float eps, void* stream) {
  if (!param || !grad || !exp_avg || !exp_avg_sq) return WGNN_ERR_NULL;
  if (n < 1 || step < 1) return WGNN_ERR_SHAPE;
  return launch_adam(param, grad, exp_avg, exp_avg_sq, n, step, lr, beta1, beta2, eps, (hipStream_t)stream);
}

}
```

### windgnn_amd/csrc/common.h

```cpp
#pragma once
#include <hip/hip_runtime.h>
#include <stdint.h>

#include "../../include/windgnn.h"

typedef float f32x4 __attribute__((ext_vector_type(4)));
typedef float f32x16 __attribute__((ext_vector_type(16)));

#define WGNN_WAVE 64

static inline int cdiv_i(int a, int b) { return (a + b - 1) / b; }
static inline size_t align_up(size_t x, size_t a) { return (x + a - 1) / a * a; }

#define WGNN_CHECK_LAUNCH()                              \
  do {                                                   \
    if (hipGetLastError() != hipSuccess) return WGNN_ERR_HIP; \
  } while (0)

__device__ __forceinline__ f32x4 mfma16(float a, float b, f32x4 c) {
  return __builtin_amdgcn_mfma_f32_16x16x4f32(a, b, c, 0, 0, 0);
}
__device__ __forceinline__ f32x16 mfma32(float a, float b, f32x16 c) {
  return __builtin_amdgcn_mfma_f32_32x32x2f32(a, b, c, 0, 0, 0);
}

__device__ __forceinline__ float sigmoidf_(float x) { return 1.0f / (1.0f + expf(-x)); }
__device__ __forceinline__ float sigmoid_fast(float x) {
  return __builtin_amdgcn_rcpf(1.0f + __builtin_amdgcn_exp2f(-1.4426950408889634f * x));
}
__device__ __forceinline__ float tanh_fast(float x) {
  return 1.0f - 2.0f * __builtin_amdgcn_rcpf(__builtin_amdgcn_exp2f(2.8853900817779268f * x) + 1.0f);
}
__device__ __forceinline__ float tanhf_(float x) {
  return 1.0f - 2.0f / (expf(2.0f * x) + 1.0f);
}

#include <atomic>
static inline int ensure_dyn_smem(const void* fn, size_t bytes, std::atomic<unsigned long long>& done) {
  int dev = 0;
  if (hipGetDevice(&dev) != hipSuccess) return WGNN_ERR_HIP;
  const unsigned long long bit = 1ull << (dev & 63);
  if (done.load(std::memory_order_acquire) & bit) return WGNN_OK;
  if (hipFuncSetAttribute(fn, hipFuncAttributeMaxDynamicSharedMemorySize, (int)bytes) != hipSuccess)
    return WGNN_ERR_HIP;
  done.fetch_or(bit, std::memory_order_release);
  return WGNN_OK;
}

void prof_begin(const char* kernel, double flops, double bytes, hipStream_t st);
void prof_end(hipStream_t st);
extern bool g_prof_on;
#define PROF_LAUNCH(name, flops, bytes, st, ...) \
  do {                                            \
    if (g_prof_on) prof_begin(name, flops, bytes, st); \
    __VA_ARGS__;                                  \
    if (g_prof_on) prof_end(st);                  \
  } while (0)

#define WGNN_FP16_MAX 65504.0f
__device__ __forceinline__ bool out_of_fp16_range(float v) { return !(__builtin_fabsf(v) <= WGNN_FP16_MAX); }
__device__ __forceinline__ void report_status(unsigned* status, bool bad, unsigned bit) {
  if (status && bad) atomicOr(status, bit);
}

struct BwdState { const float* h0; const float* dhn; float* dh0; };
template <typename... S>
__device__ __forceinline__ BwdState bwd_state(S... s) {
  if constexpr (sizeof...(S) == 0) return BwdState{nullptr, nullptr, nullptr};
  else return BwdState{s...};
}

struct SeriesRows { int stride; };
__device__ __forceinline__ BwdState bwd_state(SeriesRows) { return BwdState{nullptr, nullptr, nullptr}; }
struct SeriesStarts { const int* starts; int last; };
__device__ __forceinline__ BwdState bwd_state(SeriesStarts) { return BwdState{nullptr, nullptr, nullptr}; }
struct MaskedLabels {};
__device__ __forceinline__ BwdState bwd_state(SeriesRows, MaskedLabels) { return BwdState{nullptr, nullptr, nullptr}; }
__device__ __forceinline__ BwdState bwd_state(SeriesStarts, MaskedLabels) { return BwdState{nullptr, nullptr, nullptr}; }
struct LossFn { int kind; float delta; int t_from; int masked; };
static inline bool lossfn_valid(const LossFn& f, int T) {
  return f.kind >= 0 && f.kind <= 2 && (f.masked == 0 || f.masked == 1) && f.t_from >= 0 && f.t_from < T &&
         (f.kind != 2 || (f.delta > 0.f && f.delta < __builtin_inff()));
}
__device__ __forceinline__ BwdState bwd_state(SeriesRows, LossFn) { return BwdState{nullptr, nullptr, nullptr}; }
__device__ __forceinline__ BwdState bwd_state(SeriesStarts, LossFn) { return BwdState{nullptr, nullptr, nullptr}; }

struct GemmArgs {
  const float* A; int lda; int a_kcontig;
  const float* B; int ldb; int b_kcontig;
  float* C; int ldc;
  int M, N, K;
  const float* bias;
  int ones_col;
  int shift_T;
  int splitk;
  float* partial;
};
int launch_gemm_f32(const GemmArgs& g, hipStream_t st);
int gemm_f32_nt_splitk(int M, int N, int K);
int launch_gemm_f32_nt(GemmArgs g, float* kpart, hipStream_t st);
void gemm_f32_tile(int M, int N, int* bm, int* bn);
int gemm_f32_tiles(int M, int N);
bool gemm32_nt_supported(size_t BT, int Kp_f, int Kp_b);
bool gemm32_tn_supported(size_t BT);
int gemm32_nt_rows(int N);
int launch_pad_weight(const float* W, int R, int C, int transpose, const float* bias, float* out, int Ro, int Co,
                      hipStream_t st);
int launch_gemm32_nt(const float* A, int lda, int M, int Kp, const float* Bp, float* C, int ldc, int N, hipStream_t st);
int gemm32_tn_tiles(int Mo, int No);
int gemm32_tn_pitch(int No);
int launch_gemm32_tn(const float* A, int lda, const float* B, int ldb, int K, int splitk, float* P, int Mo, int No,
                     const float* A2, int lda2, int msplit, hipStream_t st);

int launch_mse_stats(const float* Y, const float* L, int64_t n, float grad_scale, float* loss, float* scales,
                     float* part , hipStream_t st);
int launch_amax_scale(const float* x, int64_t n, float* scales, float* part , hipStream_t st,
                      const float* x2 = nullptr, int64_t n2 = 0 );
bool grux_shape_supported(int H);
int grux_hp(int H);
size_t grux_gates_floats(int B, int T, int H, int io);
int launch_grux_fwd(int B, int T, int H, const void* GI , int ldgi, const float* Whh, const float* bhh, void* Y,
                    float* gates, void* y_planes, bool x3, unsigned* status, const void* labels, float* stat_part,
                    int io , int last_only, float y_mul, float y_add, hipStream_t st,
                    const float* h0 = nullptr ,
                    float* hn = nullptr ,
                    size_t plane_rows = 0 );
int grux_blocks(int B);
int mse_stats_blocks();
int grux_hn(int H);
int grux_msplit(int H);
int launch_grux_bwd(int B, int T, int H, const float* Whh, const void* Y, const float* dY, const void* labels, int io,
                    const float* gates, const float* GI , int ldgi,
                    const float* scales, void* dGI_planes, void* dGHn_planes, int ldd, bool x3, const float* stat_part,
                    int64_t n_loss, float grad_scale, float* loss, float* scales_out, unsigned* status,
                    int write_lo , hipStream_t st,
                    const BwdState* state = nullptr );
#define WGNN_STATS_TAG 20261004.0f
#define WGNN_STATS_TAG_MASKED 20261019.0f
#define WGNN_STATS_TAG_LOSSFN 20261030.0f
__host__ __device__ __forceinline__ unsigned* masked_counts(float* stat_part, int nb) {
  return (unsigned*)(stat_part + 2 * (size_t)nb + 4);
}
__host__ __device__ __forceinline__ const unsigned* masked_counts(const float* stat_part, int nb) {
  return (const unsigned*)(stat_part + 2 * (size_t)nb + 4);
}


int launch_gcn_partial_reduce(const float* partial, int nblk, float* dW1, float* db1, float* dW2, float* db2,
                              unsigned* status, hipStream_t st);
size_t gcn32_bwd_partial_floats(int ntiles);
int launch_gcn32_fwd(int ntiles, int S, const float* A, const float* X, const float* W1, const float* b1,
                     const float* W2, const float* b2, float* g, int ldg, float* xtail_scratch, hipStream_t st);
int launch_gcn32_bwd(int ntiles, int S, const float* A, const float* X, const float* W1, const float* b1,
                     const float* W2, const float* g, int ldg, const float* dg, int ld_dg, float* dW1, float* db1, float* dW2,
                     float* db2, float* partial, float* xtail_scratch, hipStream_t st);
size_t gcnx2_bwd_partial_floats(int ntiles);
int gcnx_bwd_grid(int ntiles, int S, bool x3);
int launch_gcnx2_fwd(int ntiles, int S, const float* A, const void* X, int io , const float* W1, const float* b1,
                     const float* W2, const float* b2, void* g_planes, int ldg, bool x3, unsigned* status, void* xtail_scratch,
                     hipStream_t st);
int launch_gcnx2_bwd(int ntiles, int S, const float* A, const void* X, int io, const float* W1, const float* b1,
                     const float* W2, const void* g_planes, int ldg, const void* dg, int ld_dg ,
                     bool dg16 , const float* scales, int scale_in, float* partial, bool x3,
                     void* xtail_scratch, hipStream_t st);
bool gcngi_supported(int S, int H, bool x3);
int launch_gcngi_fwd(int ntiles, int S, const float* A, const void* X, int io, const float* W1, const float* b1,
                     const float* W2, const float* b2, void* g_planes, int ldg, int stash_planes, const void* Bplanes,
                     int Np, void* GI, int ldgi, int N, bool x3, unsigned* status, void* xtail_scratch, hipStream_t st);
bool gcn_any_supported(int S, int Fi, int Fo);
size_t gcn_any_bwd_partial_floats(int ntiles, int Fi, int Fo);
int launch_gcn_any_fwd(int ntiles, int S, int Fi, int Fo, const float* A, const float* X, const float* W, const float* b, float* out,
                       hipStream_t st);
int launch_gcn_any_bwd(int ntiles, int S, int Fi, int Fo, const float* A, const float* X, const float* W, const float* out,
                       const float* dout, float* dW, float* db, float* dX, float* partial, hipStream_t st);
int launch_pack_g(const float* gin, size_t rows, int I, float* g, int ld, hipStream_t st);
int launch_unpack_dg(const float* dg, size_t rows, int I, int ld, float* out, hipStream_t st);
bool gcn_wide_supported(int S, int Fi, int Fo);
bool gcn_wide_countable(int ntiles, int S, int Fi, int Fo);
size_t gcn_wide_bwd_ws_floats(int ntiles, int S, int Fi, int Fo);
int launch_gcn_wide_fwd(int ntiles, int S, int Fi, int Fo, const float* A, const float* X, const float* W, const float* b,
                        float* out, hipStream_t st);
int launch_gcn_wide_bwd(int ntiles, int S, int Fi, int Fo, const float* A, const float* X, const float* W, const float* out,
                        const float* dout, float* dW, float* db, float* dX, float* ws, hipStream_t st);
bool pgemm_nt256_wanted(int M, int N, int Kp);
int launch_pgemm_nt256(const void* Aimg_hi, const void* Aimg_lo, int M, int k0, int klen, const void* Bplanes, int Np,
                       size_t bplane, float* C, int ldc, int N, bool accumulate, hipStream_t st);
size_t pgemm_nt256_aimg_bytes(int M, int N, int Kp, int planes);
int launch_pgemm_repack_a(const void* Ahi, const void* Alo, int lda, int M, int Kp, void* img, hipStream_t st);
int opt_big_gemm();
bool hh_from_y(const wgnn_dims* d, bool tn_merge, bool sst);
__host__ __device__ __forceinline__ size_t bimg_off(int n, int k, int Np) {
  return ((size_t)(k >> 5) * (size_t)(Np >> 4) + (size_t)(n >> 4)) * 512 + (size_t)(((k >> 3) & 3) * 128 + (n & 15) * 8 + (k & 7));
}
int launch_split_weight2(const float* W, int R, int C, int transpose, const float* bias, int bias_col, void* planes,
                         int Rp, int Cp, unsigned* status, hipStream_t st);
int pgemm_nt_np(int N);
int pgemm_tn_tiles(int Mout, int Nout);
size_t pgemm_tn_partial_floats(int Mout, int Nout, int splitk);
size_t pgemm_nt_kpart_floats(int M, int ldc, int Kp);
int launch_pgemm_nt(const void* Ahi, const void* Alo, int lda, int M, int Kp, const void* Bplanes, int Np, float* C,
                    int ldc, int N, const float* s_out, bool x3, float* kpart, hipStream_t st, bool out16 = false,
                    void* aimg = nullptr );
int launch_pgemm_tn(const void* Ahi, const void* Alo, int lda, const void* Bhi, const void* Blo, int ldb, int shift_T,
                    int K, int splitk, float* partial, int Mout, int Nout, bool x3, const void* A2hi, const void* A2lo,
                    int lda2, int msplit, hipStream_t st, bool b_stream = false ,
                    bool per_window = false );
struct TnProd {
  const void *Ahi, *Alo; int lda;
  const void *Bhi, *Blo; int ldb;
  int shift_T, splitk;
  float* partial;
  int Mout, Nout;
  bool x3;
  const void *A2hi, *A2lo; int lda2, msplit;
  bool b_stream, per_window;
  const float* By;
};
bool pgemm_tn2_covers(const TnProd& ih, const TnProd& hh);
TnProd tn_b_from_y(TnProd hh, const float* Y, int H);
int launch_pgemm_tn2(const TnProd& ih, const TnProd& hh, int K, hipStream_t st);
size_t gcn_csr_bwd_partial_floats();
int launch_gcn2_csr_fwd(int ntiles, int S, int nnz, const void* csr, const float* X, const float* W1, const float* b1,
                        const float* W2, const float* b2, float* h1, float* g, void* g_planes, size_t ldg, bool x3,
                        unsigned* status, hipStream_t st);
int launch_gcn2_csr_bwd(int ntiles, int S, int nnz, const void* csr, const float* X, const float* W2, const float* h1,
                        const float* g, const void* g_hi, size_t ldg, const float* dg, size_t ld_dg,
                        const float* scales, float* du, float* partial, float* dW1, float* db1, float* dW2, float* db2,
                        hipStream_t st);
int launch_gru_gen_fwd_x3(int B, int T, int H, const float* GI, int ldgi, const void* whh_planes, int np_g3,
                          const float* bhh, float* Y, float* gates, void* y_planes, float* gh, float* kpart, void* hc,
                          bool x3, hipStream_t st, const float* h0 = nullptr,
                          size_t plane_rows = 0 );
int launch_h0_planes(int B, int H, int Hp, const float* h0, void* hi, void* lo, hipStream_t st);
int launch_gru_gen_bwd_x3(int B, int T, int H, const void* whhT_planes, int np_h, const float* Y, const float* dY,
                          const float* gates, const float* scales, void* dgi_planes, void* dgh_planes, int ldd,
                          float* dhz, float* dhw, float* kpart, void* dc, bool x3, hipStream_t st,
                          const BwdState* state = nullptr);
int launch_gru_gen_fwd(int B, int T, int H, const float* GI, int ldgi, const float* Whh, const float* bhh, float* Y,
                       float* gates, float* gh, hipStream_t st, const float* h0 = nullptr);
int launch_gru_gen_bwd(int B, int T, int H, const float* Whh, const float* Y, const float* dY, const float* gates,
                       float* dGI, float* dGH, int ldd, float* dhz, float* dhw, hipStream_t st,
                       const BwdState* state = nullptr);
size_t gcn1_csr_bwd_ws_floats(int ntiles, int S);
int launch_gcn1_csr_fwd(int ntiles, int S, int nnz, const void* csr, const float* X, const float* W, const float* b,
                        float* out, hipStream_t st);
int launch_gcn1_csr_bwd(int ntiles, int S, int nnz, const void* csr, const float* X, const float* W, const float* out,
                        const float* dout, float* dW, float* db, float* dX, float* ws, hipStream_t st);
int launch_gcn1_fwd(int ntiles, int S, const float* A, const float* X, const float* W,
                    const float* b, float* out, hipStream_t st);
size_t gcn1_bwd_partial_floats(int ntiles);
int launch_gcn1_bwd(int ntiles, int S, const float* A, const float* X, const float* W,
                    const float* out, const float* dout, float* dW, float* db, float* dX,
                    float* partial, hipStream_t st);

int launch_gru_fwd(int B, int T, int H, const float* GI, int ldgi, const float* Whh, const float* bhh, float* Y,
                   float* gates, const float* labels, float* stat_part, float* hprev, int hq, int last_only, float y_mul,
                   float y_add, hipStream_t st, const float* h0 = nullptr, float* hn = nullptr,
                   int series_stride = 0 ,
                   int64_t ls_rows = 0 ,
                   const int* starts = nullptr ,
                   int starts_last = 0, bool masked = false ,
                   const LossFn* lossfn = nullptr );
int launch_gru_bwd(int B, int T, int H, const float* Whh, const float* Y, const float* dY, const float* labels,
                   const float* gates, const float* GI , int ldgi, float* dGI, int ldd, float* dGHn, float* dGH, const float* stat_part,
                   int64_t n_loss, float grad_scale, float* loss, unsigned* status, hipStream_t st,
                   const BwdState* state = nullptr ,
                   int series_stride = 0 ,
                   int64_t ls_rows = 0 ,
                   const int* starts = nullptr , int starts_last = 0,
                   bool masked = false ,
                   const LossFn* lossfn = nullptr );
bool gru_shape_supported(int H);
size_t gru_gates_floats(int B, int T, int H);
int gru_blocks(int B);
int gru_hn(int H);
int gru_msplit(int H);
bool gru_small_supported(int B, int H);
int launch_gru_small_fwd(int B, int T, int H, const float* GI, int ldgi, const float* Whh, const float* bhh, float* Y,
                         float* gates, float* hprev , int hq,
                         const float* labels , float* stat_part ,
                         hipStream_t st, const float* h0 = nullptr, float* hn = nullptr);
int gru_small_blocks(int B);
int launch_gru_small_bwd(int B, int T, int H, const float* Whh, const float* Y, const float* dY, const float* labels,
                         const float* gates, float* dGI, float* dGH, int ldd, const float* stat_part, int64_t n_loss,
                         float grad_scale, float* loss, unsigned* status, hipStream_t st,
                         const BwdState* state = nullptr );

enum { SER_NONE = 0, SER_FRONT = 1, SER_REC = 2 };
static inline size_t ser_front(int series, size_t n) { return series == SER_REC ? 0 : n; }
static inline size_t ser_rec(int series, size_t n) { return series == SER_FRONT ? 0 : n; }
struct SeriesPlan {
  size_t ws_front, ws_rec;
  size_t ws_front_fwd;
  size_t st_front, st_rec;
  size_t st_g, st_GI, st_gates, st_hprev;
};
int series_plan(const wgnn_dims* front, const wgnn_dims* rec, SeriesPlan* sp);
int series_fwd(const wgnn_dims* front, const wgnn_dims* rec, int stride, const float* A, const float* Xs, const wgnn_params* p,
               float* Y, float* last , float wind_min, float wind_max, void* stash ,
               void* workspace, const SeriesPlan& sp, void* stream, const int* starts = nullptr );
int series_bwd(const wgnn_dims* front, const wgnn_dims* rec, int stride, const float* A, const float* Xs, const wgnn_params* p,
               const float* Y, const float* dY, const void* stash, const wgnn_grads* g, void* workspace, const SeriesPlan& sp,
               void* stream, const int* starts = nullptr);
size_t series_loss_floats(int n);
size_t series_masked_loss_floats(int n);
int series_fwd_loss(const wgnn_dims* front, const wgnn_dims* rec, int stride, const float* A, const float* Xs,
                    const wgnn_params* p, const float* Ls, int64_t ls_rows, float* Y, void* stash , float* loss_buf,
                    void* workspace, const SeriesPlan& sp, void* stream, const int* starts = nullptr, bool masked = false,
                    const LossFn* lossfn = nullptr );
int series_bwd_mse(const wgnn_dims* front, const wgnn_dims* rec, int stride, const float* A, const float* Xs,
                   const wgnn_params* p, const float* Y, const float* Ls, int64_t ls_rows, float grad_scale, const void* stash,
                   const float* loss_buf, float* loss, const wgnn_grads* g, void* workspace, const SeriesPlan& sp, void* stream,
                   const int* starts = nullptr, bool masked = false, const LossFn* lossfn = nullptr);
int series_val_fwd(const wgnn_dims* front, const wgnn_dims* rec, int stride, const float* A, const float* Xs,
                   const wgnn_params* p, const float* Ls, int64_t ls_rows, float* last, float wind_min, float wind_max,
                   float* loss_buf, void* workspace, const SeriesPlan& sp, void* stream, const int* starts, const LossFn* lossfn);
int launch_series_fold(const float* dGI, int n, int T, int stride, int rows, int G3, int ld, float* dGIs, hipStream_t st);
int launch_series_fold_at(const float* dGI, const int* starts, int n, int T, int rows, int G3, int ld, float* dGIs,
                          hipStream_t st);

#define WGNN_STEP_MAX_B 256
bool gru_step_supported(int B, int S, int H);
int launch_gru_step(int B, int S, int H, const float* A, const float* X, const float* W1, const float* b1, const float* W2,
                    const float* b2, const float* Wih, const float* bih, const float* Whh, const float* bhh, const float* h0,
                    float* Y, float* hn, hipStream_t st);

int launch_mse(const float* Y, const float* L, int64_t n, float scale, float* dY, float* loss,
               float* ws, hipStream_t st);

constexpr int TN_BM = 320, TN_WAVES = 8;
void pgemm_tn_geom(int Mgemm, int Nout, int* T, int* nNb, int* ntiles);
int gcn32_bwd_grid(int ntiles, int S);
int gcn_csr_bwd_rows();
struct FinSeg {
  const float* partial;
  int splitk;
  int kind;
  int T, nNb, ntiles;
  int Mout, Nout, ncols;
  int pitch;
  int Mgemm;
  int msplit, rows1;
  int scaled;
  int nblocks;
};
struct FinishArgs {
  FinSeg ih, hh;
  const float* conv_partial;
  int conv_rows, conv_blocks, elem_blocks;
  unsigned elem_mask;
  const float* scales;
  unsigned* status;
  float* g[8];
  float* p[8];
  float* m[8];
  float* v[8];
  int n[8];
  int adam;
  float lr_over_bc1, inv_sqrt_bc2, b1, b2, eps;
  int prep_kind;
  _Float16 *pf_hi, *pf_lo, *pb_hi, *pb_lo;
  int np_g3, np_i;
  float *wp, *wt;
  int Ip, Gp, I;
  float* clip;
  float max_norm;
};
int launch_finish(FinishArgs a, hipStream_t st);
constexpr int CLIP_HDR = 64;
int finish_grid(FinishArgs& a, int64_t* grid);
int launch_finish_norm(FinishArgs a, hipStream_t st);
int launch_finish_clipped(FinishArgs a, hipStream_t st);
struct RowsAdamArgs {
  float *p_w, *m_w, *v_w;
  const float* g_w;
  float *p_b, *m_b, *v_b;
  const float* g_b;
  int row0, rows, ncols;
  float lr_over_bc1, inv_sqrt_bc2, b1, b2, eps;
  _Float16 *pf_hi, *pf_lo, *pb_hi, *pb_lo;
  int np_g3, np_i;
  unsigned* status;
  int vec;
};
int launch_adam_rows(const RowsAdamArgs& a, hipStream_t st);
int launch_adam(float* p, const float* g, float* m, float* v, int64_t n, int step, float lr,
                float b1, float b2, float eps, hipStream_t st);
```

### windgnn_amd/csrc/grux.hip

```cpp
#include "common.h"
#include <type_traits>

typedef _Float16 h8 __attribute__((ext_vector_type(8)));
typedef _Float16 h2v __attribute__((ext_vector_type(2)));
typedef float f32x2 __attribute__((ext_vector_type(2)));

namespace {

constexpr int MB = 16;
constexpr int NTHREADS = 512;
__host__ __device__ constexpr int grec(int io) { return io ? 5 : 4; }

struct Frag { h8 hi, lo; };

__device__ __forceinline__ f32x4 mfma_x(h8 a, h8 b, f32x4 c) {
  return __builtin_amdgcn_mfma_f32_16x16x32_f16(a, b, c, 0, 0, 0);
}
template <bool X3>
__device__ __forceinline__ f32x4 mfma3(const Frag& a, const Frag& b, f32x4 c) {
  if (X3) {
    c = mfma_x(a.lo, b.hi, c);
    c = mfma_x(a.hi, b.lo, c);
  }
  c = mfma_x(a.hi, b.hi, c);
  return c;
}
__device__ __forceinline__ void split2(float x0, float x1, unsigned& hi, unsigned& lo) {
  float t0, t1;
  asm("v_cvt_pk_f16_f32 %0, %4, %5\n\t"
      "v_fma_mix_f32 %2, %0, -1.0, %4 op_sel:[0,0,0] op_sel_hi:[1,0,0]\n\t"
      "v_fma_mix_f32 %3, %0, -1.0, %5 op_sel:[1,0,0] op_sel_hi:[1,0,0]\n\t"
      "v_cvt_pk_f16_f32 %1, %2, %3\n\t"
      "s_nop 1"
      : "=&v"(hi), "=&v"(lo), "=&v"(t0), "=&v"(t1)
      : "v"(x0), "v"(x1));
}
__device__ __forceinline__ Frag split_vals(const float (&x)[8]) {
  typedef unsigned int u32x4v __attribute__((ext_vector_type(4)));
  u32x4v hi, lo;
#pragma unroll
  for (int j = 0; j < 4; ++j) {
    unsigned h, l;
    split2(x[2 * j], x[2 * j + 1], h, l);
    hi[j] = h;
    lo[j] = l;
  }
  Frag f;
  f.hi = __builtin_bit_cast(h8, hi);
  f.lo = __builtin_bit_cast(h8, lo);
  return f;
}
__device__ __forceinline__ float io_load(const void* p, int idx, int io) {
  if (io == 0) return ((const float*)p)[idx];
  const unsigned short u = ((const unsigned short*)p)[idx];
  if (io == 1) return (float)__builtin_bit_cast(_Float16, u);
  return __builtin_bit_cast(float, (unsigned)u << 16);
}
__device__ __forceinline__ void io_store(void* p, int idx, float v, int io) {
  if (io == 0) { ((float*)p)[idx] = v; return; }
  if (io == 1) { ((_Float16*)p)[idx] = (_Float16)v; return; }
  ((__bf16*)p)[idx] = (__bf16)v;
}
template <bool X3>
__device__ __forceinline__ void put_split(_Float16* hi, _Float16* lo, int idx, float v) {
  const _Float16 h = (_Float16)v;
  hi[idx] = h;
  if (X3) lo[idx] = (_Float16)(v - (float)h);
}

template <int KS, bool X3, bool IO, bool ST = false>
__global__ void __launch_bounds__(NTHREADS) grux_fwd_kernel(int B, int T, int H, const void* __restrict__ GI, int ldgi,
                                                            const float* __restrict__ Whh,
                                                            const float* __restrict__ bhh, void* __restrict__ Y,
                                                            float* __restrict__ gates, _Float16* __restrict__ yp_hi,
                                                            _Float16* __restrict__ yp_lo, unsigned* status,
                                                            const void* __restrict__ Lab,
                                                            float* __restrict__ stat_part, int io, int last_only,
                                                            float y_mul, float y_add, const float* __restrict__ h0,
                                                            float* __restrict__ hn) {
  if (!ST) { h0 = nullptr; hn = nullptr; }
  constexpr int HP = 32 * KS;
  constexpr int HS = 32 * KS + 8;
  __shared__ __attribute__((aligned(16))) _Float16 hbuf[2 * 2 * MB * HS];
  bool h0bad = false;
  for (int i = threadIdx.x; i < 2 * 2 * MB * HS; i += NTHREADS) {
    const int m = (i % (MB * HS)) / HS, k = i % HS, b = blockIdx.x * MB + m;
    float v = 0.f;
    if (h0 && i < 2 * MB * HS && k < H && b < B) {
      const float x = h0[(size_t)b * H + k];
      h0bad |= out_of_fp16_range(x);
      v = i < MB * HS ? x : (X3 ? x - (float)(_Float16)x : 0.f);
    }
    hbuf[i] = (_Float16)v;
  }
  report_status(status, h0bad, WGNN_STATUS_ACT_RANGE);
  __syncthreads();
  if (threadIdx.x < 2 * MB)
    hbuf[(threadIdx.x / MB) * 2 * MB * HS + (threadIdx.x % MB) * HS + H] = (_Float16)1.f;

  if (stat_part && blockIdx.x == 0 && threadIdx.x == 0) stat_part[2 * gridDim.x] = Lab ? WGNN_STATS_TAG : 0.f;
  if (yp_hi && blockIdx.x == 0 && threadIdx.x < HP) {
    yp_hi[(size_t)B * T * HP + threadIdx.x] = (_Float16)(threadIdx.x == H ? 1.f : 0.f);
    yp_lo[(size_t)B * T * HP + threadIdx.x] = (_Float16)0.f;
  }
  const int lane = threadIdx.x & 63, wave = threadIdx.x >> 6, c = lane & 15, g = lane >> 4;
  const int j = 16 * wave + c;
  const bool active = 16 * wave < H;
  const bool jv = j < H;
  const int jc = jv ? j : H - 1;
  const int b0 = blockIdx.x * MB;

  bool wbad = false;
  Frag WB[3][KS];
#pragma unroll
  for (int gate = 0; gate < 3; ++gate)
#pragma unroll
    for (int ks = 0; ks < KS; ++ks) {
      float x[8];
#pragma unroll
      for (int jj = 0; jj < 8; ++jj) {
        const int k = 32 * ks + 8 * g + jj;
        x[jj] = (jv && k < H) ? Whh[(size_t)(gate * H + j) * H + k] : 0.f;
        wbad |= out_of_fp16_range(x[jj]);
      }
      WB[gate][ks] = split_vals(x);
    }
  if (blockIdx.x == 0) report_status(status, wbad, WGNN_STATUS_WEIGHT_RANGE);
  const float bh_r = bhh[jc], bh_z = bhh[H + jc], bh_n = bhh[2 * H + jc];

  typedef typename std::conditional<X3, float, _Float16>::type gi_t;
  const gi_t* GIw = (const gi_t*)GI + (size_t)b0 * T * ldgi;
  constexpr int esz = IO ? 2 : 4;
  void* Yw = (char*)Y + (size_t)b0 * T * H * esz;
  const int NW = (H + 15) / 16;
  constexpr int GREC = X3 ? (IO ? 4 : 3) : (IO ? 3 : 2);
  f32x4* gatesw = gates ? (f32x4*)gates + ((size_t)blockIdx.x * T * NW + wave) * GREC * 64 + lane : nullptr;
  int rowt[4];
  bool rowok[4];
#pragma unroll
  for (int r = 0; r < 4; ++r) {
    const int m = 4 * g + r;
    rowok[r] = jv && b0 + m < B;
    rowt[r] = (b0 + m < B ? m : B - 1 - b0) * T;
  }
  constexpr int HY = HP + 2;
  __shared__ __attribute__((aligned(16))) float ytile[IO ? 2 * MB * HY : 4];
  __shared__ __attribute__((aligned(16))) float ltile[IO ? 2 * MB * HY : 4];
  const int UPR = (H + 1) / 2;
  constexpr int NU = (MB * (HP / 2) + NTHREADS - 1) / NTHREADS;
  int u_lds[NU], u_glb[NU], u_n[NU];
#pragma unroll
  for (int i = 0; i < NU; ++i) {
    const int q = threadIdx.x + NTHREADS * i;
    const int m = q / UPR, e = 2 * (q % UPR);
    const bool ok = q < MB * UPR && b0 + m < B;
    u_lds[i] = ok ? m * HY + e : 0;
    u_glb[i] = ok ? m * T * H + e : 0;
    u_n[i] = ok ? (e + 1 < H ? 2 : 1) : 0;
  }
  const void* Labw = Lab ? (const char*)Lab + (size_t)b0 * T * H * esz : nullptr;
  f32x2 lraw[NU];
  auto load_lab = [&](int t) {
    if (!IO || !Lab) return;
    const int tc = t < T ? t : T - 1;
#pragma unroll
    for (int i = 0; i < NU; ++i) {
      const int o = u_glb[i] + tc * H;
      if (io == 0) {
        if (u_n[i] == 2) lraw[i] = *(const f32x2*)((const float*)Labw + o);
        else if (u_n[i] == 1) lraw[i][0] = ((const float*)Labw)[o];
      } else {
        if (u_n[i] == 2) lraw[i][0] = __builtin_bit_cast(float, *(const unsigned*)((const unsigned short*)Labw + o));
        else if (u_n[i] == 1) lraw[i][0] = __builtin_bit_cast(float, (unsigned)((const unsigned short*)Labw)[o]);
      }
    }
  };
  auto stage_lab = [&](int t) {
    if (!IO || !Lab) return;
    float* lt = ltile + (t & 1) * MB * HY;
#pragma unroll
    for (int i = 0; i < NU; ++i) {
      if (u_n[i] == 0) continue;
      f32x2 v = lraw[i];
      if (io == 1) {
        v = __builtin_convertvector(__builtin_bit_cast(h2v, __builtin_bit_cast(unsigned, lraw[i][0])), f32x2);
      } else if (io == 2) {
        const unsigned u = __builtin_bit_cast(unsigned, lraw[i][0]);
        v[0] = __builtin_bit_cast(float, u << 16);
        v[1] = __builtin_bit_cast(float, u & 0xffff0000u);
      }
      lt[u_lds[i]] = v[0];
      if (u_n[i] == 2) lt[u_lds[i] + 1] = v[1];
    }
  };
  float ssum = 0.f, smax = 0.f;
  float lab[4] = {0.f, 0.f, 0.f, 0.f}, labn[4] = {0.f, 0.f, 0.f, 0.f};
  float gi[3][4], gin[3][4];
  auto load_gi = [&](int t, float (&dst)[3][4], float (&ldst)[4]) {
    const int tc = t < T ? t : T - 1;
#pragma unroll
    for (int r = 0; r < 4; ++r) {
      const int o = (rowt[r] + tc) * ldgi + jc;
      dst[0][r] = (float)GIw[o];
      dst[1][r] = (float)GIw[o + H];
      dst[2][r] = (float)GIw[o + 2 * H];
      if (!IO && Lab) ldst[r] = ((const float*)Labw)[(rowt[r] + tc) * H + jc];
    }
  };
  load_lab(0);
  stage_lab(0);
  load_gi(0, gi, lab);
  float hold[4] = {0.f, 0.f, 0.f, 0.f};
  if (h0) {
#pragma unroll
    for (int r = 0; r < 4; ++r) hold[r] = rowok[r] ? h0[(size_t)(b0 + 4 * g + r) * H + j] : 0.f;
  }
  __syncthreads();

  for (int t = 0; t < T; ++t) {
    const _Float16* hhi = hbuf + (t & 1) * 2 * MB * HS;
    const _Float16* hlo = hhi + MB * HS;
    _Float16* nhi = hbuf + ((t + 1) & 1) * 2 * MB * HS;
    _Float16* nlo = nhi + MB * HS;
    load_gi(t + 1, gin, labn);
    load_lab(t + 1);
    float* yt = ytile + (t & 1) * MB * HY;
    const float* lt = ltile + (t & 1) * MB * HY;
    float hnew[4] = {0.f, 0.f, 0.f, 0.f};
    if (active) {
      f32x4 ar, az, an;
#pragma unroll
      for (int r = 0; r < 4; ++r) {
        ar[r] = gi[0][r] + bh_r;
        az[r] = gi[1][r] + bh_z;
        an[r] = bh_n;
      }
#pragma unroll
      for (int ks = 0; ks < KS; ++ks) {
        Frag a;
        a.hi = *(const h8*)(hhi + c * HS + 32 * ks + 8 * g);
        if (X3) a.lo = *(const h8*)(hlo + c * HS + 32 * ks + 8 * g);
        else a.lo = a.hi;
        ar = mfma3<X3>(a, WB[0][ks], ar);
        az = mfma3<X3>(a, WB[1][ks], az);
        an = mfma3<X3>(a, WB[2][ks], an);
      }
      f32x4 rg4, zg4, ng4;
#pragma unroll
      for (int r = 0; r < 4; ++r) {
        const float rg = sigmoid_fast(ar[r]);
        const float zg = sigmoid_fast(az[r]);
        const float ng = tanh_fast(__builtin_fmaf(rg, an[r], gi[2][r]));
        rg4[r] = rg; zg4[r] = zg; ng4[r] = ng;
        hnew[r] = (1.f - zg) * ng + zg * hold[r];
        hold[r] = hnew[r];
      }
#pragma unroll
      for (int r = 0; r < 4; ++r) {
        if (IO) {
          if (jv) yt[(4 * g + r) * HY + j] = hnew[r];
        } else if (rowok[r]) {
          if (!last_only) ((float*)Yw)[(rowt[r] + t) * H + j] = hnew[r];
          else if (t == T - 1) ((float*)Y)[(size_t)(b0 + 4 * g + r) * H + j] = hnew[r] * y_mul + y_add;
        }
        if (hn && rowok[r] && t == T - 1) hn[(size_t)(b0 + 4 * g + r) * H + j] = hnew[r];
        if (rowok[r] && Lab) {
          const float dl = hnew[r] - (IO ? lt[(4 * g + r) * HY + j] : lab[r]);
          ssum = fmaf(dl, dl, ssum);
          smax = fmaxf(smax, fabsf(dl));
        }
      }
      if (gates) {
        f32x4* rec = gatesw + (size_t)t * NW * GREC * 64;
        if (X3) {
          rec[0] = rg4;
          rec[64] = zg4;
          rec[128] = an;
        } else {
          h8 rz, ng;
#pragma unroll
          for (int r = 0; r < 4; ++r) {
            rz[r] = (_Float16)rg4[r];
            rz[4 + r] = (_Float16)zg4[r];
            ng[r] = (_Float16)ng4[r];
            ng[4 + r] = (_Float16)an[r];
          }
          rec[0] = __builtin_bit_cast(f32x4, rz);
          rec[64] = __builtin_bit_cast(f32x4, ng);
        }
        if (IO) {
          const f32x4 h4 = {hnew[0], hnew[1], hnew[2], hnew[3]};
          rec[(GREC - 1) * 64] = h4;
        }
      }
    }
    if (active) {
#pragma unroll
      for (int r = 0; r < 4; ++r) put_split<X3>(nhi, nlo, (4 * g + r) * HS + (jv ? j : HP + (c & 7)), hnew[r]);
    }
    stage_lab(t + 1);
    __syncthreads();
#pragma unroll
    for (int i = 0; i < (IO ? NU : 0); ++i) {
      if (ST && !Y) break;
      if (u_n[i] == 0) continue;
      const float v0 = yt[u_lds[i]], v1 = yt[u_lds[i] + 1];
      const int o = u_glb[i] + t * H;
      if (io == 0) {
        if (u_n[i] == 2) { const f32x2 v = {v0, v1}; *(f32x2*)((float*)Yw + o) = v; }
        else ((float*)Yw)[o] = v0;
      } else {
        unsigned pk;
        if (io == 1) {
          const f32x2 v = {v0, v1};
          pk = __builtin_bit_cast(unsigned, __builtin_convertvector(v, h2v));
        } else {
          typedef __bf16 bf2 __attribute__((ext_vector_type(2)));
          const f32x2 v = {v0, v1};
          pk = __builtin_bit_cast(unsigned, __builtin_convertvector(v, bf2));
        }
        if (u_n[i] == 2) *(unsigned*)((unsigned short*)Yw + o) = pk;
        else ((unsigned short*)Yw)[o] = (unsigned short)pk;
      }
    }
    if (yp_hi) {
      for (int q = threadIdx.x; q < (X3 ? 2 : 1) * MB * (HP / 8); q += NTHREADS) {
        const int plane = q / (MB * (HP / 8)), rem = q % (MB * (HP / 8));
        const int m = rem / (HP / 8), ch = rem % (HP / 8);
        const int b = b0 + m;
        if (b < B) {
          const h8 v = *(const h8*)((plane ? nlo : nhi) + m * HS + 8 * ch);
          __builtin_nontemporal_store(v, (h8*)((plane ? yp_lo : yp_hi) + (size_t)b0 * T * HP + (m * T + t) * HP + 8 * ch));
        }
      }
    }
#pragma unroll
    for (int q = 0; q < 3; ++q)
#pragma unroll
      for (int r = 0; r < 4; ++r) gi[q][r] = gin[q][r];
#pragma unroll
    for (int r = 0; r < 4; ++r) lab[r] = labn[r];
  }
  if (Lab) {
    __shared__ float red[2][NTHREADS / 64];
#pragma unroll
    for (int o = 32; o > 0; o >>= 1) {
      ssum += __shfl_xor(ssum, o, 64);
      smax = fmaxf(smax, __shfl_xor(smax, o, 64));
    }
    if (lane == 0) {
      red[0][wave] = ssum;
      red[1][wave] = smax;
    }
    __syncthreads();
    if (threadIdx.x == 0) {
      float a = 0.f, m = 0.f;
#pragma unroll
      for (int w = 0; w < NTHREADS / 64; ++w) {
        a += red[0][w];
        m = fmaxf(m, red[1][w]);
      }
      stat_part[blockIdx.x] = a;
      stat_part[gridDim.x + blockIdx.x] = m;
    }
  }
}

template <int KSB, bool X3, bool IO, typename... St>
__global__ void __launch_bounds__(NTHREADS) grux_bwd_kernel(int B, int T, int H, const float* __restrict__ Whh,
                                                            const void* __restrict__ Y, const float* __restrict__ dY,
                                                            const void* __restrict__ Lab, int io,
                                                            const float* __restrict__ gates,
                                                            const float* __restrict__ GIn, int ldgi,
                                                            const float* __restrict__ scales,
                                                            _Float16* __restrict__ dGI_hi, _Float16* __restrict__ dGI_lo,
                                                            int ldd, _Float16* __restrict__ dGN_hi,
                                                            _Float16* __restrict__ dGN_lo,
                                                            const float* __restrict__ stat_part, int nstat, float inv_n,
                                                            float coef_in, float* __restrict__ loss_out,
                                                            float* __restrict__ scales_out, unsigned* status,
                                                            int write_lo, St... state) {
  constexpr bool ST = sizeof...(St) > 0;
  const BwdState sb = bwd_state(state...);
  constexpr int DS = 32 * KSB + 24;
  float s_fin = 1.f, c_fin = coef_in;
  if (stat_part) {
    __shared__ float sred[2][NTHREADS / 64];
    float a = 0.f, m = 0.f;
    for (int i = threadIdx.x; i < nstat; i += NTHREADS) {
      a += stat_part[i];
      m = fmaxf(m, stat_part[nstat + i]);
    }
#pragma unroll
    for (int o = 32; o > 0; o >>= 1) {
      a += __shfl_xor(a, o, 64);
      m = fmaxf(m, __shfl_xor(m, o, 64));
    }
    if ((threadIdx.x & 63) == 0) {
      sred[0][threadIdx.x >> 6] = a;
      sred[1][threadIdx.x >> 6] = m;
    }
    __syncthreads();
    a = 0.f;
    m = 0.f;
#pragma unroll
    for (int w = 0; w < NTHREADS / 64; ++w) {
      a += sred[0][w];
      m = fmaxf(m, sred[1][w]);
    }
    const bool tagged = stat_part[2 * nstat] == WGNN_STATS_TAG;
    m *= fabsf(coef_in);
    if (m > 0.f && m < 3.0e38f) {
      int e;
      frexpf(m, &e);
      s_fin = ldexpf(1.f, 1 - e);
    }
    if (blockIdx.x == 0 && threadIdx.x == 0) {
      loss_out[0] = tagged ? a * inv_n : __builtin_nanf("");
      scales_out[0] = s_fin;
      scales_out[1] = 1.f / s_fin;
      scales_out[2] = coef_in;
      if (!tagged && status) atomicOr(status, WGNN_STATUS_NO_LOSS_STATS);
    }
  }
  __shared__ __attribute__((aligned(16))) _Float16 dbuf2[2 * 4 * MB * DS];
  for (int i = threadIdx.x; i < 2 * 4 * MB * DS; i += NTHREADS) dbuf2[i] = (_Float16)0.f;

  const int lane = threadIdx.x & 63, wave = threadIdx.x >> 6, c = lane & 15, g = lane >> 4;
  const int j = 16 * wave + c;
  const bool active = 16 * wave < H;
  const bool jv = j < H;
  const int jc = jv ? j : H - 1;
  const int b0 = blockIdx.x * MB;
  const int MS = 8 * ((2 * H + 7) / 8), HN = 8 * ((H + 7) / 8);
  const float s_in = stat_part ? s_fin : (scales ? scales[0] : 1.f);
  const float coef = stat_part ? c_fin : (Lab ? scales[2] : 1.f);

  Frag WT[KSB];
#pragma unroll
  for (int ks = 0; ks < KSB; ++ks) {
    float x[8];
#pragma unroll
    for (int jj = 0; jj < 8; ++jj) {
      const int k = 32 * ks + 8 * g + jj;
      const int row = k < 2 * H ? k : ((k >= MS && k - MS < H) ? 2 * H + (k - MS) : -1);
      x[jj] = (jv && row >= 0) ? Whh[(size_t)row * H + j] : 0.f;
    }
    WT[ks] = split_vals(x);
  }
  const int NW = (H + 15) / 16;
  const f32x4* gatesw = (const f32x4*)gates + ((size_t)blockIdx.x * T * NW + (active ? wave : 0)) * (X3 ? (IO ? 4 : 3) : (IO ? 3 : 2)) * 64 + lane;
  constexpr int esz = IO ? 2 : 4;
  constexpr int GREC = X3 ? (IO ? 4 : 3) : (IO ? 3 : 2);
  const float* GIw = X3 ? GIn + (size_t)b0 * T * ldgi + 2 * H : nullptr;
  const void* Labw = Lab ? (const char*)Lab + (size_t)b0 * T * H * esz : nullptr;
  const float* dYw = dY ? dY + (size_t)b0 * T * H : nullptr;
  const float* Yw = (const float*)Y + (size_t)b0 * T * H;
  int rowt[4];
  bool rowok[4];
#pragma unroll
  for (int r = 0; r < 4; ++r) {
    const int m = 4 * g + r;
    rowok[r] = jv && b0 + m < B;
    rowt[r] = (b0 + m < B ? m : B - 1 - b0) * T;
  }
  constexpr int NCH = (2 * MB * (4 * KSB) + 2 * MB * (4 * KSB) / 2 + NTHREADS - 1) / NTHREADS;
  int c_lds[NCH], c_step[NCH];
  _Float16* c_dst[NCH];
  {
    const int cpr = ldd / 8, cpn = HN / 8;
    const int n_i = 2 * MB * cpr, n_n = 2 * MB * cpn;
#pragma unroll
    for (int i = 0; i < NCH; ++i) {
      int q = threadIdx.x + NTHREADS * i;
      c_dst[i] = nullptr;
      c_lds[i] = 0;
      c_step[i] = 0;
      if (q < n_i) {
        const int plane = q / (MB * cpr), rem = q % (MB * cpr), m = rem / cpr, ch = rem % cpr;
        if (b0 + m < B && ((X3 && write_lo) || plane == 0)) {
          c_lds[i] = (2 + plane) * MB * DS + m * DS + 8 * ch;
          c_dst[i] = (plane ? dGI_lo : dGI_hi) + ((size_t)(b0 + m) * T) * ldd + 8 * ch;
          c_step[i] = ldd;
        }
      } else if (q - n_i < n_n) {
        q -= n_i;
        const int plane = q / (MB * cpn), rem = q % (MB * cpn), m = rem / cpn, ch = rem % cpn;
        if (b0 + m < B && ((X3 && write_lo) || plane == 0)) {
          c_lds[i] = plane * MB * DS + m * DS + MS + 8 * ch;
          c_dst[i] = (plane ? dGN_lo : dGN_hi) + ((size_t)(b0 + m) * T) * HN + 8 * ch;
          c_step[i] = HN;
        }
      }
    }
  }
  constexpr int HY = 32 * ((KSB * 32 / 3 + 31) / 32) + 34;
  __shared__ __attribute__((aligned(16))) float ltile[IO ? 2 * MB * HY : 4];
  const int UPR = (H + 1) / 2;
  constexpr int NU = IO ? (MB * (HY / 2) + NTHREADS - 1) / NTHREADS : 1;
  int u_lds[NU], u_glb[NU], u_n[NU];
#pragma unroll
  for (int i = 0; i < NU; ++i) {
    const int q = threadIdx.x + NTHREADS * i;
    const int m = q / UPR, e = 2 * (q % UPR);
    const bool ok = IO && Lab && q < MB * UPR && b0 + m < B;
    u_lds[i] = ok ? m * HY + e : 0;
    u_glb[i] = ok ? m * T * H + e : 0;
    u_n[i] = ok ? (e + 1 < H ? 2 : 1) : 0;
  }
  f32x2 lraw[NU];
  auto load_lab = [&](int t) {
    const int tc = t > 0 ? t : 0;
#pragma unroll
    for (int i = 0; i < NU; ++i) {
      const int o = u_glb[i] + tc * H;
      if (io == 0) {
        if (u_n[i] == 2) lraw[i] = *(const f32x2*)((const float*)Labw + o);
        else if (u_n[i] == 1) lraw[i][0] = ((const float*)Labw)[o];
      } else {
        if (u_n[i] == 2) lraw[i][0] = __builtin_bit_cast(float, *(const unsigned*)((const unsigned short*)Labw + o));
        else if (u_n[i] == 1) lraw[i][0] = __builtin_bit_cast(float, (unsigned)((const unsigned short*)Labw)[o]);
      }
    }
  };
  auto stage_lab = [&](int t) {
    float* lt = ltile + (t & 1) * MB * HY;
#pragma unroll
    for (int i = 0; i < NU; ++i) {
      if (u_n[i] == 0) continue;
      f32x2 v = lraw[i];
      if (io == 1) {
        v = __builtin_convertvector(__builtin_bit_cast(h2v, __builtin_bit_cast(unsigned, lraw[i][0])), f32x2);
      } else if (io == 2) {
        const unsigned u = __builtin_bit_cast(unsigned, lraw[i][0]);
        v[0] = __builtin_bit_cast(float, u << 16);
        v[1] = __builtin_bit_cast(float, u & 0xffff0000u);
      }
      lt[u_lds[i]] = v[0];
      if (u_n[i] == 2) lt[u_lds[i] + 1] = v[1];
    }
  };
  float h0r[4] = {0.f, 0.f, 0.f, 0.f};
  float s_out = 1.f;
  if constexpr (ST) {
#pragma unroll
    for (int r = 0; r < 4; ++r) h0r[r] = sb.h0[(size_t)(b0 + rowt[r] / T) * H + jc];
    s_out = scales ? scales[1] : 1.f;
  }
  struct StepIn { float dy[4], r[4], z[4], n[4], ghn[4], hp[4]; };
  auto load_step = [&](int t, StepIn& s) {
    const int tc = t > 0 ? t : 0;
    const f32x4* rec = gatesw + (size_t)tc * NW * GREC * 64;
    f32x4 r4, z4, n4, g4;
    if (X3) {
      r4 = rec[0]; z4 = rec[64]; g4 = rec[128];
#pragma unroll
      for (int r = 0; r < 4; ++r) n4[r] = GIw[(rowt[r] + tc) * ldgi + jc];
    } else {
      const h8 rz = __builtin_bit_cast(h8, rec[0]), ng = __builtin_bit_cast(h8, rec[64]);
#pragma unroll
      for (int r = 0; r < 4; ++r) {
        r4[r] = (float)rz[r];
        z4[r] = (float)rz[4 + r];
        n4[r] = (float)ng[r];
        g4[r] = (float)ng[4 + r];
      }
    }
#pragma unroll
    for (int r = 0; r < 4; ++r) {
      const int bt = rowt[r] + tc;
      s.dy[r] = Lab ? (IO ? 0.f : ((const float*)Labw)[bt * H + jc]) : dYw[bt * H + jc];
      s.r[r] = r4[r];
      s.z[r] = z4[r];
      s.n[r] = n4[r];
      s.ghn[r] = g4[r];
      const float hp = IO ? 0.f : Yw[(bt - (tc > 0 ? 1 : 0)) * H + jc];
      s.hp[r] = tc > 0 ? hp : 0.f;
      if constexpr (ST) {
        if (tc == 0) s.hp[r] = h0r[r];
      }
    }
    if (IO && tc > 0) {
      const f32x4 h4 = (gatesw + (size_t)(tc - 1) * NW * GREC * 64)[(GREC - 1) * 64];
#pragma unroll
      for (int r = 0; r < 4; ++r) s.hp[r] = h4[r];
    }
  };
  StepIn cur, nxt;
  load_step(T - 1, cur);
  float ycur[4] = {0.f, 0.f, 0.f, 0.f};
  if (Lab) {
    if (IO) {
      const f32x4 h4 = (gatesw + (size_t)(T - 1) * NW * GREC * 64)[(GREC - 1) * 64];
#pragma unroll
      for (int r = 0; r < 4; ++r) ycur[r] = h4[r];
    } else {
#pragma unroll
      for (int r = 0; r < 4; ++r) ycur[r] = Yw[(rowt[r] + T - 1) * H + jc];
    }
    if (IO) {
      load_lab(T - 1);
      stage_lab(T - 1);
    }
  }
  f32x4 dhn = {0.f, 0.f, 0.f, 0.f};
  if (ST && sb.dhn) {
#pragma unroll
    for (int r = 0; r < 4; ++r) dhn[r] = rowok[r] ? sb.dhn[(size_t)(b0 + 4 * g + r) * H + j] * s_in : 0.f;
  }
  const int o_pad = 32 * KSB + 8 + (c & 7);
  const int o_r = jv ? j : o_pad, o_z = jv ? H + j : o_pad, o_n = jv ? MS + j : o_pad, o_t = jv ? 2 * H + j : o_pad;
  __syncthreads();

  for (int t = T - 1; t >= 0; --t) {
    _Float16* dbuf = dbuf2 + (t & 1) * 4 * MB * DS;
    _Float16* dhi = dbuf;
    _Float16* dlo = dbuf + MB * DS;
    _Float16* ihi = dbuf + 2 * MB * DS;
    _Float16* ilo = dbuf + 3 * MB * DS;
    load_step(t - 1, nxt);
    if (IO && Lab) load_lab(t - 1);
    const float* lt = ltile + (t & 1) * MB * HY;
    f32x4 acc = {0.f, 0.f, 0.f, 0.f};
    if (active) {
#pragma unroll
      for (int r = 0; r < 4; ++r) {
        const int m = 4 * g + r;
        const float dyv = Lab ? (ycur[r] - (IO ? lt[m * HY + jc] : cur.dy[r])) * coef : cur.dy[r];
        const float dh = rowok[r] ? dyv * s_in + dhn[r] : 0.f;
        const float rg = cur.r[r], zg = cur.z[r];
        const float ng = X3 ? tanh_fast(__builtin_fmaf(rg, cur.ghn[r], cur.n[r])) : cur.n[r];
        const float dn = dh * (1.f - zg);
        const float dz = dh * (cur.hp[r] - ng);
        const float dnt = dn * (1.f - ng * ng);
        const float dr = dnt * cur.ghn[r];
        const float dar = dr * rg * (1.f - rg);
        const float daz = dz * zg * (1.f - zg);
        const float dnr = dnt * rg;
        acc[r] = dh * zg;
        const _Float16 arh = (_Float16)dar, azh = (_Float16)daz, nrh = (_Float16)dnr, nth = (_Float16)dnt;
        dhi[m * DS + o_r] = arh;
        dhi[m * DS + o_z] = azh;
        dhi[m * DS + o_n] = nrh;
        ihi[m * DS + o_r] = arh;
        ihi[m * DS + o_z] = azh;
        ihi[m * DS + o_t] = nth;
        if (X3) {
          const _Float16 arl = (_Float16)(dar - (float)arh), azl = (_Float16)(daz - (float)azh);
          dlo[m * DS + o_r] = arl;
          dlo[m * DS + o_z] = azl;
          dlo[m * DS + o_n] = (_Float16)(dnr - (float)nrh);
          ilo[m * DS + o_r] = arl;
          ilo[m * DS + o_z] = azl;
          ilo[m * DS + o_t] = (_Float16)(dnt - (float)nth);
        }
      }
    }
    if (IO && Lab) stage_lab(t - 1);
    __syncthreads();
#pragma unroll
    for (int i = 0; i < NCH; ++i) {
      if (c_dst[i]) {
        const h8 v = *(const h8*)(dbuf + c_lds[i]);
        *(h8*)(c_dst[i] + (size_t)t * c_step[i]) = v;
      }
    }
    if (active && (ST || t > 0)) {
#pragma unroll
      for (int ks = 0; ks < KSB; ++ks) {
        Frag a;
        a.hi = *(const h8*)(dhi + c * DS + 32 * ks + 8 * g);
        if (X3) a.lo = *(const h8*)(dlo + c * DS + 32 * ks + 8 * g);
        else a.lo = a.hi;
        acc = mfma3<X3>(a, WT[ks], acc);
      }
      if (ST && t == 0 && sb.dh0) {
#pragma unroll
        for (int r = 0; r < 4; ++r)
          if (rowok[r]) sb.dh0[(size_t)(b0 + 4 * g + r) * H + j] = acc[r] * s_out;
      }
    }
    dhn = acc;
    __syncthreads();
#pragma unroll
    for (int r = 0; r < 4; ++r) ycur[r] = cur.hp[r];
    cur = nxt;
  }
}

}

bool grux_shape_supported(int H) { return H >= 1 && H <= 127; }

int grux_hp(int H) { return 32 * cdiv_i(H + 1, 32); }
size_t grux_gates_floats(int B, int T, int H, int io) {
  return (size_t)cdiv_i(B, MB) * T * cdiv_i(H, 16) * grec(io) * 64 * 4;
}
int grux_blocks(int B) { return cdiv_i(B, MB); }
static double gates_bytes(int B, int T, int H, int io, bool x3) {
  return (double)cdiv_i(B, MB) * T * cdiv_i(H, 16) * (x3 ? (io ? 4 : 3) : (io ? 3 : 2)) * 64 * 16.0;
}

int launch_grux_fwd(int B, int T, int H, const void* GI , int ldgi, const float* Whh, const float* bhh, void* Y,
                    float* gates, void* y_planes , bool x3, unsigned* status,
                    const void* labels , float* stat_part , int io,
                    int last_only ,
                    float y_mul, float y_add, hipStream_t st, const float* h0, float* hn, size_t plane_rows) {
  if (last_only && (io != 0 || gates || y_planes || labels)) return WGNN_ERR_UNSUPPORTED;
  if (!Y && (!io || !hn || last_only)) return WGNN_ERR_NULL;
  _Float16* yh = (_Float16*)y_planes;
  _Float16* yl = yh ? yh + (plane_rows ? plane_rows : (size_t)B * T + 1) * grux_hp(H) : nullptr;
  const double bt = (double)B * T;
  const double fl = bt * 2.0 * 3 * H * H,
               by = bt * ((x3 ? 4.0 : 2.0) * 3 * H + (io ? 2.0 : 4.0) * ((last_only ? 0 : H) + (labels ? H : 0))) +
                    (gates ? gates_bytes(B, T, H, io, x3) : 0.0);
  const dim3 grid(cdiv_i(B, MB));
#define FLAUNCH(K, X3V, IOV, NAME)                                                                                 \
  PROF_LAUNCH(NAME, fl, by, st,                                                                                    \
              if (h0 || hn) hipLaunchKernelGGL((grux_fwd_kernel<K, X3V, IOV, true>), grid, dim3(NTHREADS), 0, st, B, T, H, GI,  \
                                               ldgi, Whh, bhh, Y, gates, yh, yl, status, labels, stat_part, io, last_only,     \
                                               y_mul, y_add, h0, hn);                                                          \
              else hipLaunchKernelGGL((grux_fwd_kernel<K, X3V, IOV, false>), grid, dim3(NTHREADS), 0, st, B, T, H, GI, ldgi,   \
                                      Whh, bhh, Y, gates, yh, yl, status, labels, stat_part, io, last_only, y_mul, y_add,      \
                                      nullptr, nullptr))
#define FCASE(K)                                                                                                   \
  if (x3 && !io) FLAUNCH(K, true, false, "grux_fwd_kernel<" #K ">");                                               \
  else if (x3) FLAUNCH(K, true, true, "grux_fwd_kernel<" #K ">");                                                  \
  else if (!io) FLAUNCH(K, false, false, "grux_fwd_kernel<" #K ",f16>");                                           \
  else FLAUNCH(K, false, true, "grux_fwd_kernel<" #K ",f16>")
  switch (cdiv_i(H + 1, 32)) {
    case 1: FCASE(1); break;
    case 2: FCASE(2); break;
    case 3: FCASE(3); break;
    case 4: FCASE(4); break;
    default: return WGNN_ERR_UNSUPPORTED;
  }
#undef FCASE
#undef FLAUNCH
  WGNN_CHECK_LAUNCH();
  return WGNN_OK;
}

int grux_hn(int H) { return 8 * cdiv_i(H, 8); }
int grux_msplit(int H) { return 8 * cdiv_i(2 * H, 8); }

int launch_grux_bwd(int B, int T, int H, const float* Whh, const void* Y, const float* dY, const void* labels, int io,
                    const float* gates, const float* GI , int ldgi,
                    const float* scales, void* dGI_planes, void* dGHn_planes, int ldd, bool x3, const float* stat_part,
                    int64_t n_loss, float grad_scale, float* loss, float* scales_out, unsigned* status, int write_lo,
                    hipStream_t st, const BwdState* state) {
  if (state && (!state->h0 || labels || stat_part)) return WGNN_ERR_UNSUPPORTED;
  const int nstat = grux_blocks(B);
  const float inv_n = stat_part ? 1.0f / (float)n_loss : 0.f, coef_in = stat_part ? 2.0f * grad_scale / (float)n_loss : 0.f;
  _Float16* ih = (_Float16*)dGI_planes;
  _Float16* il = ih + (size_t)B * T * ldd;
  _Float16* nh = (_Float16*)dGHn_planes;
  _Float16* nl = nh + (size_t)B * T * grux_hn(H);
  const int ksb = cdiv_i(grux_msplit(H) + H, 32);
  if (ldd % 8 != 0 || ldd < 3 * H || ldd > 32 * ksb) return WGNN_ERR_SHAPE;
  if (x3 && (!GI || ldgi < 3 * H)) return WGNN_ERR_NULL;
  const double bt = (double)B * T;
  const double fl = bt * 2.0 * 3 * H * H,
               by = bt * ((io ? 2.0 + 4.0 : 4.0 + 4.0) * H + (x3 && write_lo ? 4.0 : 2.0) * (3 * H + H)) +
                    gates_bytes(B, T, H, io, x3) + (x3 ? bt * 4.0 * H : 0.0);
  const dim3 grid(cdiv_i(B, MB));
#define BLAUNCH(K, X3V, IOV, NAME, BYTES)                                                                         \
  PROF_LAUNCH(NAME, fl, BYTES, st,                                                                                \
              if (state) hipLaunchKernelGGL((grux_bwd_kernel<K, X3V, IOV, BwdState>), grid, dim3(NTHREADS), 0, st, B, T, H, Whh, Y, dY, \
                                            labels, io, gates, GI, ldgi, scales, ih, il, ldd, nh, nl, stat_part, nstat, inv_n, coef_in, \
                                            loss, scales_out, status, write_lo, *state);                                            \
              else hipLaunchKernelGGL((grux_bwd_kernel<K, X3V, IOV>), grid, dim3(NTHREADS), 0, st, B, T, H, Whh, Y, dY, labels, io, \
                                 gates, GI, ldgi, scales, ih, il, ldd, nh, nl, stat_part, nstat, inv_n, coef_in, loss, scales_out, status, write_lo))
#define BCASE(K)                                                                                                  \
  if (x3 && !io) BLAUNCH(K, true, false, "grux_bwd_kernel<" #K ">", by);                                          \
  else if (x3) BLAUNCH(K, true, true, "grux_bwd_kernel<" #K ">", by);                                             \
  else if (!io) BLAUNCH(K, false, false, "grux_bwd_kernel<" #K ",f16>", by);                                      \
  else BLAUNCH(K, false, true, "grux_bwd_kernel<" #K ",f16>", by)
  switch (ksb) {
    case 1: BCASE(1); break;
    case 2: BCASE(2); break;
    case 3: BCASE(3); break;
    case 4: BCASE(4); break;
    case 5: BCASE(5); break;
    case 6: BCASE(6); break;
    case 7: BCASE(7); break;
    case 8: BCASE(8); break;
    case 9: BCASE(9); break;
    case 10: BCASE(10); break;
    case 11: BCASE(11); break;
    case 12: BCASE(12); break;
    default: return WGNN_ERR_UNSUPPORTED;
  }
#undef BCASE
#undef BLAUNCH
  WGNN_CHECK_LAUNCH();
  return WGNN_OK;
}
```

Baseline: 5.558 million windows/s.

## Recompute GRU gh_n in backward instead of stashing it from forward

In the stateless fp32-I/O split-fp16 GRU path, the forward kernel no longer stores the W_hn·h+b_hn pre-activation (gh_n) in the per-step gate record, which shrinks that record from three to two f32x4 slots. The backward kernel rebuilds gh_n each step: it reads h_{t-1} from Y, splits it into hi/lo fp16 tiles in double-buffered shared memory, and runs an extra 3-pass MFMA product against the n-gate weights. This trades gate-stash memory traffic for extra matrix work, added LDS and registers, and an extra Y load per step in the serial backward recurrence. The path is on by default and can be disabled with an environment variable.

```diff
diff --git a/windgnn_amd/csrc/api.hip b/windgnn_amd/csrc/api.hip
--- a/windgnn_amd/csrc/api.hip
+++ b/windgnn_amd/csrc/api.hip
@@ -36,7 +36,7 @@
   size_t st_h1;
   size_t st_stats;
   size_t st_GI;
-  bool gi_stash;
+  bool gi_stash, ghn_rc;
   size_t ws_gh, ws_h1, ws_yp, ws_hhp_f, ws_kp_f, ws_hc, ws_du, ws_dhz, ws_dhw, ws_hhp_b, ws_kp_b, ws_dc;
   size_t ws_ntk_f, ws_ntk_b;
   size_t ws_aimg_f, ws_aimg_b;
@@ -119,7 +119,7 @@
     const size_t nb = L.small ? (size_t)gru_small_blocks(d->B) : (size_t)grux_blocks(d->B);
     L.st_stats = o; o += al(series ? 0 : 2 * nb + 4);
   }
-  L.gi_stash = (x3 && !L.gen_gru && three_pass(d)) || L.rec32;
+  L.gi_stash = (x3 && !L.gen_gru && three_pass(d)) || L.rec32; L.ghn_rc = !series && !L.gen_gru && ghn_recompute(d, state);
   L.st_GI = o; o += al(ser_front(series, L.gi_stash ? L.BT * L.Gp : 0));
   L.hq = (int)rup(L.H + 1, 16);
   const bool hprev_rows = L.g32tn || (state && !x3);
@@ -448,7 +448,7 @@
     }
     rc = launch_grux_fwd(d->B, d->T, d->H, f.GI, (int)L.Gp, p->w_hh, p->b_hh, f.Y, f.gates,
                          f.sf && !hh_from_y(d, L.tn_merge, c.sst) ? f.sf + L.st_yp : nullptr, f.full, f.status, labels, stats,
-                         d->io, 0, 1.f, 0.f, f.st, c.h0, c.hn, c.sst ? L.plane_rows : 0);
+                         d->io, 0, 1.f, 0.f, f.st, c.h0, c.hn, c.sst ? L.plane_rows : 0, L.ghn_rc);
   } else if (L.rec32) {
     if (c.last)
       return launch_gru_fwd(d->B, d->T, d->H, f.GI, (int)L.Gp, p->w_hh, p->b_hh, c.last, nullptr, nullptr, nullptr, nullptr, 0,
@@ -603,7 +603,7 @@
     return launch_grux_bwd(d->B, d->T, d->H, p->w_hh, c.Y, b.fused_loss ? nullptr : dY, b.fused_loss ? c.labels : nullptr,
                            d->io, gates, L.gi_stash ? b.sf + L.st_GI : nullptr, (int)L.Gp, b.scales, b.dGI, b.dGH, (int)L.Gp,
                            b.full, stats, (int64_t)L.BT * L.H, c.grad_scale, c.loss, b.scales, b.status, L.dgi1 ? 0 : 1, b.st,
-                           sb);
+                           sb, p->b_hh, L.ghn_rc);
   }
   if (L.gen_gru)
     return launch_gru_gen_bwd(d->B, d->T, d->H, p->w_hh, b.Y, dY, gates, b.dGI, b.dGH, (int)L.Gp, b.ws + L.ws_dhz,
@@ -812,6 +812,10 @@
   return tn_merge && three_pass(d) && d->io == WGNN_IO_F32 && !sst && from_env && opt(WGNN_OPT_TN_MERGED);
 }
 
+bool ghn_recompute(const wgnn_dims* d, bool sst) {
+  return three_pass(d) && grux_shape_supported(d->H) && d->io == WGNN_IO_F32 && !sst && env_int("WGNN_GHN_RECOMPUTE", 1, 0, 1);
+}
+
 int series_plan(const wgnn_dims* df, const wgnn_dims* dr, SeriesPlan* sp) {
   int rc = check_dims(df);
   if (rc == WGNN_OK) rc = check_dims(dr);
diff --git a/windgnn_amd/csrc/common.h b/windgnn_amd/csrc/common.h
--- a/windgnn_amd/csrc/common.h
+++ b/windgnn_amd/csrc/common.h
@@ -124,7 +124,8 @@
                     int io , int last_only, float y_mul, float y_add, hipStream_t st,
                     const float* h0 = nullptr ,
                     float* hn = nullptr ,
-                    size_t plane_rows = 0 );
+                    size_t plane_rows = 0 ,
+                    bool ghn_rc = false );
 int grux_blocks(int B);
 int mse_stats_blocks();
 int grux_hn(int H);
@@ -134,7 +135,8 @@
                     const float* scales, void* dGI_planes, void* dGHn_planes, int ldd, bool x3, const float* stat_part,
                     int64_t n_loss, float grad_scale, float* loss, float* scales_out, unsigned* status,
                     int write_lo , hipStream_t st,
-                    const BwdState* state = nullptr );
+                    const BwdState* state = nullptr ,
+                    const float* bhh = nullptr, bool ghn_rc = false );
 #define WGNN_STATS_TAG 20261004.0f
 #define WGNN_STATS_TAG_MASKED 20261019.0f
 #define WGNN_STATS_TAG_LOSSFN 20261030.0f
@@ -189,6 +191,7 @@
 int launch_pgemm_repack_a(const void* Ahi, const void* Alo, int lda, int M, int Kp, void* img, hipStream_t st);
 int opt_big_gemm();
 bool hh_from_y(const wgnn_dims* d, bool tn_merge, bool sst);
+bool ghn_recompute(const wgnn_dims* d, bool sst);
 __host__ __device__ __forceinline__ size_t bimg_off(int n, int k, int Np) {
   return ((size_t)(k >> 5) * (size_t)(Np >> 4) + (size_t)(n >> 4)) * 512 + (size_t)(((k >> 3) & 3) * 128 + (n & 15) * 8 + (k & 7));
 }
diff --git a/windgnn_amd/csrc/grux.hip b/windgnn_amd/csrc/grux.hip
--- a/windgnn_amd/csrc/grux.hip
+++ b/windgnn_amd/csrc/grux.hip
@@ -67,8 +67,39 @@
   hi[idx] = h;
   if (X3) lo[idx] = (_Float16)(v - (float)h);
 }
-
-template <int KS, bool X3, bool IO, bool ST = false>
+template <int KS>
+__device__ __forceinline__ bool whh_gate_frags(const float* __restrict__ Whh, int H, int gate, int j, bool jv, int g,
+                                               Frag (&W)[KS]) {
+  bool bad = false;
+#pragma unroll
+  for (int ks = 0; ks < KS; ++ks) {
+    float x[8];
+#pragma unroll
+    for (int jj = 0; jj < 8; ++jj) {
+      const int k = 32 * ks + 8 * g + jj;
+      x[jj] = (jv && k < H) ? Whh[(size_t)(gate * H + j) * H + k] : 0.f;
+      bad |= out_of_fp16_range(x[jj]);
+    }
+    W[ks] = split_vals(x);
+  }
+  return bad;
+}
+template <int KS, bool X3, int NG>
+__device__ __forceinline__ void hh_product(const _Float16* hhi, const _Float16* hlo, int c, int g, const Frag (*W)[KS],
+                                           f32x4 (&acc)[NG]) {
+  constexpr int HS = 32 * KS + 8;
+#pragma unroll
+  for (int ks = 0; ks < KS; ++ks) {
+    Frag a;
+    a.hi = *(const h8*)(hhi + c * HS + 32 * ks + 8 * g);
+    if (X3) a.lo = *(const h8*)(hlo + c * HS + 32 * ks + 8 * g);
+    else a.lo = a.hi;
+#pragma unroll
+    for (int q = 0; q < NG; ++q) acc[q] = mfma3<X3>(a, W[q][ks], acc[q]);
+  }
+}
+
+template <int KS, bool X3, bool IO, bool ST = false, bool RC = false>
 __global__ void __launch_bounds__(NTHREADS) grux_fwd_kernel(int B, int T, int H, const void* __restrict__ GI, int ldgi,
                                                             const float* __restrict__ Whh,
                                                             const float* __restrict__ bhh, void* __restrict__ Y,
@@ -78,6 +109,7 @@
                                                             float* __restrict__ stat_part, int io, int last_only,
                                                             float y_mul, float y_add, const float* __restrict__ h0,
                                                             float* __restrict__ hn) {
+  static_assert(!RC || (X3 && !IO && !ST), "gh_n is recomputed in the stateless fp32-I/O split step only");
   if (!ST) { h0 = nullptr; hn = nullptr; }
   constexpr int HP = 32 * KS;
   constexpr int HS = 32 * KS + 8;
@@ -113,18 +145,7 @@
   bool wbad = false;
   Frag WB[3][KS];
 #pragma unroll
-  for (int gate = 0; gate < 3; ++gate)
-#pragma unroll
-    for (int ks = 0; ks < KS; ++ks) {
-      float x[8];
-#pragma unroll
-      for (int jj = 0; jj < 8; ++jj) {
-        const int k = 32 * ks + 8 * g + jj;
-        x[jj] = (jv && k < H) ? Whh[(size_t)(gate * H + j) * H + k] : 0.f;
-        wbad |= out_of_fp16_range(x[jj]);
-      }
-      WB[gate][ks] = split_vals(x);
-    }
+  for (int gate = 0; gate < 3; ++gate) wbad |= whh_gate_frags<KS>(Whh, H, gate, j, jv, g, WB[gate]);
   if (blockIdx.x == 0) report_status(status, wbad, WGNN_STATUS_WEIGHT_RANGE);
   const float bh_r = bhh[jc], bh_z = bhh[H + jc], bh_n = bhh[2 * H + jc];
 
@@ -133,7 +154,7 @@
   constexpr int esz = IO ? 2 : 4;
   void* Yw = (char*)Y + (size_t)b0 * T * H * esz;
   const int NW = (H + 15) / 16;
-  constexpr int GREC = X3 ? (IO ? 4 : 3) : (IO ? 3 : 2);
+  constexpr int GREC = X3 ? (IO ? 4 : (RC ? 2 : 3)) : (IO ? 3 : 2);
   f32x4* gatesw = gates ? (f32x4*)gates + ((size_t)blockIdx.x * T * NW + wave) * GREC * 64 + lane : nullptr;
   int rowt[4];
   bool rowok[4];
@@ -228,23 +249,15 @@
     const float* lt = ltile + (t & 1) * MB * HY;
     float hnew[4] = {0.f, 0.f, 0.f, 0.f};
     if (active) {
-      f32x4 ar, az, an;
+      f32x4 acc[3];
 #pragma unroll
       for (int r = 0; r < 4; ++r) {
-        ar[r] = gi[0][r] + bh_r;
-        az[r] = gi[1][r] + bh_z;
-        an[r] = bh_n;
-      }
-#pragma unroll
-      for (int ks = 0; ks < KS; ++ks) {
-        Frag a;
-        a.hi = *(const h8*)(hhi + c * HS + 32 * ks + 8 * g);
-        if (X3) a.lo = *(const h8*)(hlo + c * HS + 32 * ks + 8 * g);
-        else a.lo = a.hi;
-        ar = mfma3<X3>(a, WB[0][ks], ar);
-        az = mfma3<X3>(a, WB[1][ks], az);
-        an = mfma3<X3>(a, WB[2][ks], an);
-      }
+        acc[0][r] = gi[0][r] + bh_r;
+        acc[1][r] = gi[1][r] + bh_z;
+        acc[2][r] = bh_n;
+      }
+      hh_product<KS, X3, 3>(hhi, hlo, c, g, WB, acc);
+      const f32x4 ar = acc[0], az = acc[1], an = acc[2];
       f32x4 rg4, zg4, ng4;
 #pragma unroll
       for (int r = 0; r < 4; ++r) {
@@ -275,7 +288,7 @@
         if (X3) {
           rec[0] = rg4;
           rec[64] = zg4;
-          rec[128] = an;
+          if (!RC) rec[128] = an;
         } else {
           h8 rz, ng;
 #pragma unroll
@@ -366,7 +379,7 @@
   }
 }
 
-template <int KSB, bool X3, bool IO, typename... St>
+template <int KSB, bool X3, bool IO, int KSF, typename... St>
 __global__ void __launch_bounds__(NTHREADS) grux_bwd_kernel(int B, int T, int H, const float* __restrict__ Whh,
                                                             const void* __restrict__ Y, const float* __restrict__ dY,
                                                             const void* __restrict__ Lab, int io,
@@ -379,8 +392,10 @@
                                                             const float* __restrict__ stat_part, int nstat, float inv_n,
                                                             float coef_in, float* __restrict__ loss_out,
                                                             float* __restrict__ scales_out, unsigned* status,
-                                                            int write_lo, St... state) {
+                                                            int write_lo, const float* __restrict__ bhh, St... state) {
   constexpr bool ST = sizeof...(St) > 0;
+  constexpr bool RC = KSF > 0;
+  static_assert(!RC || (X3 && !IO && !ST), "gh_n is recomputed in the stateless fp32-I/O split step only");
   const BwdState sb = bwd_state(state...);
   constexpr int DS = 32 * KSB + 24;
   float s_fin = 1.f, c_fin = coef_in;
@@ -425,6 +440,13 @@
   }
   __shared__ __attribute__((aligned(16))) _Float16 dbuf2[2 * 4 * MB * DS];
   for (int i = threadIdx.x; i < 2 * 4 * MB * DS; i += NTHREADS) dbuf2[i] = (_Float16)0.f;
+  constexpr int HPF = 32 * KSF, HSF = 32 * KSF + 8;
+  __shared__ __attribute__((aligned(16))) _Float16 htile2[RC ? 2 * 2 * MB * HSF : 8];
+  if (RC) {
+    for (int i = threadIdx.x; i < 2 * 2 * MB * HSF; i += NTHREADS)
+      htile2[i] = (_Float16)((i % (2 * MB * HSF) < MB * HSF && i % HSF == H) ? 1.f : 0.f);
+    __syncthreads();
+  }
 
   const int lane = threadIdx.x & 63, wave = threadIdx.x >> 6, c = lane & 15, g = lane >> 4;
   const int j = 16 * wave + c;
@@ -448,10 +470,16 @@
     }
     WT[ks] = split_vals(x);
   }
+  Frag WN[1][RC ? KSF : 1];
+  float bh_n = 0.f;
+  if constexpr (RC) {
+    whh_gate_frags<KSF>(Whh, H, 2, j, jv, g, WN[0]);
+    bh_n = bhh[2 * H + jc];
+  }
+  constexpr int GREC = X3 ? (IO ? 4 : (RC ? 2 : 3)) : (IO ? 3 : 2);
   const int NW = (H + 15) / 16;
-  const f32x4* gatesw = (const f32x4*)gates + ((size_t)blockIdx.x * T * NW + (active ? wave : 0)) * (X3 ? (IO ? 4 : 3) : (IO ? 3 : 2)) * 64 + lane;
+  const f32x4* gatesw = (const f32x4*)gates + ((size_t)blockIdx.x * T * NW + (active ? wave : 0)) * GREC * 64 + lane;
   constexpr int esz = IO ? 2 : 4;
-  constexpr int GREC = X3 ? (IO ? 4 : 3) : (IO ? 3 : 2);
   const float* GIw = X3 ? GIn + (size_t)b0 * T * ldgi + 2 * H : nullptr;
   const void* Labw = Lab ? (const char*)Lab + (size_t)b0 * T * H * esz : nullptr;
   const float* dYw = dY ? dY + (size_t)b0 * T * H : nullptr;
@@ -551,9 +579,10 @@
   auto load_step = [&](int t, StepIn& s) {
     const int tc = t > 0 ? t : 0;
     const f32x4* rec = gatesw + (size_t)tc * NW * GREC * 64;
-    f32x4 r4, z4, n4, g4;
+    f32x4 r4, z4, n4, g4 = {0.f, 0.f, 0.f, 0.f};
     if (X3) {
-      r4 = rec[0]; z4 = rec[64]; g4 = rec[128];
+      r4 = rec[0]; z4 = rec[64];
+      if (!RC) g4 = rec[128];
 #pragma unroll
       for (int r = 0; r < 4; ++r) n4[r] = GIw[(rowt[r] + tc) * ldgi + jc];
     } else {
@@ -574,7 +603,7 @@
       s.z[r] = z4[r];
       s.n[r] = n4[r];
       s.ghn[r] = g4[r];
-      const float hp = IO ? 0.f : Yw[(bt - (tc > 0 ? 1 : 0)) * H + jc];
+      const float hp = (IO || RC) ? 0.f : Yw[(bt - (tc > 0 ? 1 : 0)) * H + jc];
       s.hp[r] = tc > 0 ? hp : 0.f;
       if constexpr (ST) {
         if (tc == 0) s.hp[r] = h0r[r];
@@ -586,8 +615,34 @@
       for (int r = 0; r < 4; ++r) s.hp[r] = h4[r];
     }
   };
+  auto load_hprev = [&](int s, float (&hp)[4]) {
+    const int sc = s > 0 ? s : 0;
+#pragma unroll
+    for (int r = 0; r < 4; ++r) {
+      const float v = Yw[(rowt[r] + sc - (sc > 0 ? 1 : 0)) * H + jc];
+      hp[r] = sc > 0 ? v : 0.f;
+    }
+  };
+  auto put_hprev = [&](int s, const float (&hp)[4]) {
+    _Float16* thi = htile2 + (s & 1) * 2 * MB * HSF;
+#pragma unroll
+    for (int r = 0; r < 4; ++r) put_split<true>(thi, thi + MB * HSF, (4 * g + r) * HSF + (jv ? j : HPF + (c & 7)), hp[r]);
+  };
+  auto ghn_of = [&](int s, float (&ghn)[4]) {
+    const _Float16* thi = htile2 + (s & 1) * 2 * MB * HSF;
+    f32x4 a[1] = {{bh_n, bh_n, bh_n, bh_n}};
+    hh_product<RC ? KSF : 1, true, 1>(thi, thi + MB * HSF, c, g, WN, a);
+#pragma unroll
+    for (int r = 0; r < 4; ++r) ghn[r] = a[0][r];
+  };
   StepIn cur, nxt;
   load_step(T - 1, cur);
+  float hq[4] = {0.f, 0.f, 0.f, 0.f};
+  if (RC) {
+    load_hprev(T - 1, cur.hp);
+    load_hprev(T - 2, hq);
+    if (active) put_hprev(T - 1, cur.hp);
+  }
   float ycur[4] = {0.f, 0.f, 0.f, 0.f};
   if (Lab) {
     if (IO) {
@@ -611,6 +666,7 @@
   const int o_pad = 32 * KSB + 8 + (c & 7);
   const int o_r = jv ? j : o_pad, o_z = jv ? H + j : o_pad, o_n = jv ? MS + j : o_pad, o_t = jv ? 2 * H + j : o_pad;
   __syncthreads();
+  if (RC && active) ghn_of(T - 1, cur.ghn);
 
   for (int t = T - 1; t >= 0; --t) {
     _Float16* dbuf = dbuf2 + (t & 1) * 4 * MB * DS;
@@ -619,6 +675,11 @@
     _Float16* ihi = dbuf + 2 * MB * DS;
     _Float16* ilo = dbuf + 3 * MB * DS;
     load_step(t - 1, nxt);
+    if (RC) {
+#pragma unroll
+      for (int r = 0; r < 4; ++r) nxt.hp[r] = hq[r];
+      load_hprev(t - 2, hq);
+    }
     if (IO && Lab) load_lab(t - 1);
     const float* lt = ltile + (t & 1) * MB * HY;
     f32x4 acc = {0.f, 0.f, 0.f, 0.f};
@@ -655,6 +716,7 @@
           ilo[m * DS + o_t] = (_Float16)(dnt - (float)nth);
         }
       }
+      if (RC && t > 0) put_hprev(t - 1, nxt.hp);
     }
     if (IO && Lab) stage_lab(t - 1);
     __syncthreads();
@@ -679,6 +741,7 @@
         for (int r = 0; r < 4; ++r)
           if (rowok[r]) sb.dh0[(size_t)(b0 + 4 * g + r) * H + j] = acc[r] * s_out;
       }
+      if (RC && t > 0) ghn_of(t - 1, nxt.ghn);
     }
     dhn = acc;
     __syncthreads();
@@ -697,15 +760,24 @@
   return (size_t)cdiv_i(B, MB) * T * cdiv_i(H, 16) * grec(io) * 64 * 4;
 }
 int grux_blocks(int B) { return cdiv_i(B, MB); }
-static double gates_bytes(int B, int T, int H, int io, bool x3) {
-  return (double)cdiv_i(B, MB) * T * cdiv_i(H, 16) * (x3 ? (io ? 4 : 3) : (io ? 3 : 2)) * 64 * 16.0;
+static double gates_bytes(int B, int T, int H, int io, bool x3, bool rc = false ) {
+  return (double)cdiv_i(B, MB) * T * cdiv_i(H, 16) * (x3 ? (io ? 4 : (rc ? 2 : 3)) : (io ? 3 : 2)) * 64 * 16.0;
+}
+constexpr int ghn_ksb(int H) { return (8 * ((2 * H + 7) / 8) + H + 31) / 32; }
+constexpr int ghn_ksf(int K, bool hi) {
+  int v = 0;
+  for (int H = 1; H <= 127; ++H)
+    if (ghn_ksb(H) == K && (v == 0 || hi)) v = (H + 32) / 32;
+  return v;
 }
 
 int launch_grux_fwd(int B, int T, int H, const void* GI , int ldgi, const float* Whh, const float* bhh, void* Y,
                     float* gates, void* y_planes , bool x3, unsigned* status,
                     const void* labels , float* stat_part , int io,
                     int last_only ,
-                    float y_mul, float y_add, hipStream_t st, const float* h0, float* hn, size_t plane_rows) {
+                    float y_mul, float y_add, hipStream_t st, const float* h0, float* hn, size_t plane_rows, bool ghn_rc) {
+  const bool rc = ghn_rc && gates;
+  if (rc && (!x3 || io || h0 || hn)) return WGNN_ERR_UNSUPPORTED;
   if (last_only && (io != 0 || gates || y_planes || labels)) return WGNN_ERR_UNSUPPORTED;
   if (!Y && (!io || !hn || last_only)) return WGNN_ERR_NULL;
   _Float16* yh = (_Float16*)y_planes;
@@ -713,7 +785,7 @@
   const double bt = (double)B * T;
   const double fl = bt * 2.0 * 3 * H * H,
                by = bt * ((x3 ? 4.0 : 2.0) * 3 * H + (io ? 2.0 : 4.0) * ((last_only ? 0 : H) + (labels ? H : 0))) +
-                    (gates ? gates_bytes(B, T, H, io, x3) : 0.0);
+                    (gates ? gates_bytes(B, T, H, io, x3, rc) : 0.0);
   const dim3 grid(cdiv_i(B, MB));
 #define FLAUNCH(K, X3V, IOV, NAME)                                                                                 \
   PROF_LAUNCH(NAME, fl, by, st,                                                                                    \
@@ -724,7 +796,11 @@
                                       Whh, bhh, Y, gates, yh, yl, status, labels, stat_part, io, last_only, y_mul, y_add,      \
                                       nullptr, nullptr))
 #define FCASE(K)                                                                                                   \
-  if (x3 && !io) FLAUNCH(K, true, false, "grux_fwd_kernel<" #K ">");                                               \
+  if (rc) PROF_LAUNCH("grux_fwd_kernel<" #K ">", fl, by, st,                                                       \
+                      hipLaunchKernelGGL((grux_fwd_kernel<K, true, false, false, true>), grid, dim3(NTHREADS), 0, st, B, T, H, \
+                                         GI, ldgi, Whh, bhh, Y, gates, yh, yl, status, labels, stat_part, io, last_only, y_mul,  \
+                                         y_add, nullptr, nullptr));                                                             \
+  else if (x3 && !io) FLAUNCH(K, true, false, "grux_fwd_kernel<" #K ">");                                          \
   else if (x3) FLAUNCH(K, true, true, "grux_fwd_kernel<" #K ">");                                                  \
   else if (!io) FLAUNCH(K, false, false, "grux_fwd_kernel<" #K ",f16>");                                           \
   else FLAUNCH(K, false, true, "grux_fwd_kernel<" #K ",f16>")
@@ -748,8 +824,10 @@
                     const float* gates, const float* GI , int ldgi,
                     const float* scales, void* dGI_planes, void* dGHn_planes, int ldd, bool x3, const float* stat_part,
                     int64_t n_loss, float grad_scale, float* loss, float* scales_out, unsigned* status, int write_lo,
-                    hipStream_t st, const BwdState* state) {
+                    hipStream_t st, const BwdState* state, const float* bhh, bool ghn_rc) {
   if (state && (!state->h0 || labels || stat_part)) return WGNN_ERR_UNSUPPORTED;
+  if (ghn_rc && (!x3 || io || state || !bhh)) return WGNN_ERR_UNSUPPORTED;
+  const int ksf = cdiv_i(H + 1, 32);
   const int nstat = grux_blocks(B);
   const float inv_n = stat_part ? 1.0f / (float)n_loss : 0.f, coef_in = stat_part ? 2.0f * grad_scale / (float)n_loss : 0.f;
   _Float16* ih = (_Float16*)dGI_planes;
@@ -762,17 +840,25 @@
   const double bt = (double)B * T;
   const double fl = bt * 2.0 * 3 * H * H,
                by = bt * ((io ? 2.0 + 4.0 : 4.0 + 4.0) * H + (x3 && write_lo ? 4.0 : 2.0) * (3 * H + H)) +
-                    gates_bytes(B, T, H, io, x3) + (x3 ? bt * 4.0 * H : 0.0);
+                    gates_bytes(B, T, H, io, x3, ghn_rc) + (x3 ? bt * 4.0 * H : 0.0);
   const dim3 grid(cdiv_i(B, MB));
 #define BLAUNCH(K, X3V, IOV, NAME, BYTES)                                                                         \
   PROF_LAUNCH(NAME, fl, BYTES, st,                                                                                \
-              if (state) hipLaunchKernelGGL((grux_bwd_kernel<K, X3V, IOV, BwdState>), grid, dim3(NTHREADS), 0, st, B, T, H, Whh, Y, dY, \
+              if (state) hipLaunchKernelGGL((grux_bwd_kernel<K, X3V, IOV, 0, BwdState>), grid, dim3(NTHREADS), 0, st, B, T, H, Whh, Y, dY, \
                                             labels, io, gates, GI, ldgi, scales, ih, il, ldd, nh, nl, stat_part, nstat, inv_n, coef_in, \
-                                            loss, scales_out, status, write_lo, *state);                                            \
-              else hipLaunchKernelGGL((grux_bwd_kernel<K, X3V, IOV>), grid, dim3(NTHREADS), 0, st, B, T, H, Whh, Y, dY, labels, io, \
-                                 gates, GI, ldgi, scales, ih, il, ldd, nh, nl, stat_part, nstat, inv_n, coef_in, loss, scales_out, status, write_lo))
+                                            loss, scales_out, status, write_lo, bhh, *state);                                       \
+              else hipLaunchKernelGGL((grux_bwd_kernel<K, X3V, IOV, 0>), grid, dim3(NTHREADS), 0, st, B, T, H, Whh, Y, dY, labels, io, \
+                                 gates, GI, ldgi, scales, ih, il, ldd, nh, nl, stat_part, nstat, inv_n, coef_in, loss, scales_out, status, write_lo, bhh))
+#define BLAUNCH_RC(K, KSFV)                                                                                       \
+  PROF_LAUNCH("grux_bwd_kernel<" #K ">", fl, by, st,                                                              \
+              hipLaunchKernelGGL((grux_bwd_kernel<K, true, false, KSFV>), grid, dim3(NTHREADS), 0, st, B, T, H, Whh, Y, dY, labels, \
+                                 io, gates, GI, ldgi, scales, ih, il, ldd, nh, nl, stat_part, nstat, inv_n, coef_in, loss, scales_out, \
+                                 status, write_lo, bhh))
 #define BCASE(K)                                                                                                  \
-  if (x3 && !io) BLAUNCH(K, true, false, "grux_bwd_kernel<" #K ">", by);                                          \
+  if (ghn_rc && ksf == ghn_ksf(K, false)) BLAUNCH_RC(K, ghn_ksf(K, false));                                       \
+  else if (ghn_rc && ksf == ghn_ksf(K, true)) BLAUNCH_RC(K, ghn_ksf(K, true));                                    \
+  else if (ghn_rc) return WGNN_ERR_UNSUPPORTED;                                                                   \
+  else if (x3 && !io) BLAUNCH(K, true, false, "grux_bwd_kernel<" #K ">", by);                                     \
   else if (x3) BLAUNCH(K, true, true, "grux_bwd_kernel<" #K ">", by);                                             \
   else if (!io) BLAUNCH(K, false, false, "grux_bwd_kernel<" #K ",f16>", by);                                      \
   else BLAUNCH(K, false, true, "grux_bwd_kernel<" #K ",f16>", by)
@@ -792,6 +878,7 @@
     default: return WGNN_ERR_UNSUPPORTED;
   }
 #undef BCASE
+#undef BLAUNCH_RC
 #undef BLAUNCH
   WGNN_CHECK_LAUNCH();
   return WGNN_OK;
```

Result: faster. 5.615 million windows/s (median of 6 runs) (+1.0%).
